# uoo723/PMGT

Hardware: AMD Instinct MI355X
Metric: PMGT pre-train nodes/sec (higher is better)
Workload: dtype bf16; 1 GPU; c2: 7252 nodes / 88606 edges, L=4 H=8 d=256 I=256 S=32 (context=S tokens incl. target), B=1024 targets/GPU/step, 12 sequences/target, dropout 0.1, beta 0.5, clip 5.0, AdamW lr 1e-4 wd 1e-2; parallelism=dp1, global_batch=1024, seq_len=32

## Files before the change

include/pmgt_ops.h:

```cpp
#ifndef PMGT_OPS_H
#define PMGT_OPS_H

#include "pmgt_capi.h"

#ifdef __cplusplus
extern "C" {
#endif

#define PMGT_OPT_TILE_GEMM (1u << 0)
#define PMGT_OPT_VALU_ATTENTION (1u << 1)
#define PMGT_OPT_WAVE_ATTENTION_BWD (1u << 2)
#define PMGT_OPT_NO_SHORTCUT (1u << 3)
#define PMGT_OPT_NO_FUSED_QKVC_ATTENTION (1u << 4)
#define PMGT_OPT_NO_HEAD_MAJOR (1u << 5)
#define PMGT_OPT_NO_TABLE_PROJECTION (1u << 6)
#define PMGT_OPT_NO_SEGMENT_SUM (1u << 7)
#define PMGT_OPT_CONSUMER_QUANT (1u << 8)
#define PMGT_OPT_NO_FUSED_ATTENTION_BWD (1u << 9)
#define PMGT_OPT_STORE_LN_INPUT (1u << 10)
#define PMGT_OPT_EAGER_REDUCE (1u << 11)
#define PMGT_OPT_SIDE_STREAM_REDUCE (1u << 12)
#define PMGT_OPT_UNFUSED_LN (1u << 13)
#define PMGT_OPT_ONE_BUCKET (1u << 14)
#define PMGT_OPT_SMALL_ARENA (1u << 15)
#define PMGT_OPT_NO_ROLE_SPLIT_LN (1u << 16)
#define PMGT_OPT_UNFUSED_LN_BWD (1u << 18)
#define PMGT_OPT_LOCKSTEP_ATTENTION_BWD (1u << 19)
#define PMGT_OPT_SIDE_STREAM_WGRAD (1u << 20)
#define PMGT_OPT_NO_CLS_ONLY_ATTENTION_BWD (1u << 21)
#define PMGT_OPT_NO_BETA_SKIP (1u << 22)
#define PMGT_OPT_NO_VC2_ATTENTION_BWD (1u << 23)
#define PMGT_OPT_NO_TILE_ATTENTION (1u << 17)

void pmgt_launch_trace_reset(void);
int64_t pmgt_launch_trace_count(const char* family);

int pmgt_op_clock_probe(uint64_t* out, int blocks, void* stream);
int64_t pmgt_op_seg_sort_temp_bytes(int M);
int pmgt_op_seg_sort(const int64_t* ids, int M, int n_rows, uint32_t* scratch_keys, uint32_t* scratch_vals, uint32_t* skeys, uint32_t* perm,
                     int* seg_off, void* temp, int64_t temp_bytes, void* stream);
int pmgt_op_quant_rows_e4m3(int src_dtype, const void* src, int64_t lds, int rows, int cols, void* dst, int64_t ldd,
                            float* scale, void* stream);
int pmgt_op_gemm_nt_f8(const void* A, int64_t lda, const int64_t* a_rows, const float* a_row_scale, float a_scale,
                       const void* B, int64_t ldb, const float* b_row_scale, void* C, int64_t ldc, int M, int N, int K,
                       const float* bias, const int* m_dev, void* stream);
int pmgt_op_gemm_tn_f8(const void* P, int64_t ldp, const void* Q8, int64_t ldq, float q_scale, const int64_t* q_rows, int M,
                       int N1, int N2, float* slab, float* out, int accumulate, const int* m_dev, void* stream);
int pmgt_op_qkvc_attention_fwd_f8(const void* x, const void* x8, const float* xscale, const void* w8, const float* wscale, const float* bias, const float* mask,
                                  void* qkvc, void* ctx, int n_seq, int S, int H, int dh, float beta, float drop_p,
                                  uint32_t site1, uint32_t site2, const uint64_t* rng, void* stream);
int pmgt_op_gemm_nt(int dtype, const void* A, int64_t lda, const int64_t* a_rows, const void* B, int64_t ldb, void* C,
                    int64_t ldc, int M, int N, int K, const float* bias, int epilogue, void* aux, int64_t ldaux,
                    const void* residual, int64_t ldr, float drop_p, uint32_t drop_site, const uint64_t* rng,
                    const int* m_dev, uint32_t path_opts, void* stream);
int64_t pmgt_op_gemm_tn_slab_elems(int dtype, int M, int N1, int N2, uint32_t path_opts);
int pmgt_op_gemm_tn(int dtype, const void* P, int64_t ldp, const void* Q, int64_t ldq, const int64_t* q_rows, int M,
                    int N1, int N2, float* slab, float* out, int accumulate, const int* m_dev, uint32_t path_opts, void* stream);
int pmgt_op_gemm_tn_bias(int dtype, const void* P, int64_t ldp, const void* Q, int64_t ldq, int M, int N1, int N2, float* slab,
                         float* out, float* bias_slab, float* bias_out, int perm_d, int perm_dh, uint32_t path_opts, void* stream);
int pmgt_op_colsum(int dtype, const void* Y, int64_t ldy, int M, int N, float* slab, float* out, void* stream);
int pmgt_op_layernorm_fwd(int dtype, const void* x, void* y, float* stats, const float* gamma, const float* beta,
                          int M, int d, float eps, float drop_p, uint32_t drop_site, const uint64_t* rng, void* stream);
int pmgt_op_layernorm_bwd(int dtype, const void* dy, const void* x, const float* stats, const float* gamma, void* dx,
                          void* dx_drop, float* part, float* dgamma_dbeta, int M, int d, float in_drop_p,
                          uint32_t in_site, float out_drop_p, uint32_t out_site, const uint64_t* rng, void* stream);
int pmgt_op_linear(int dtype, const void* A, int64_t lda, const void* B, int64_t ldb, void* C, int64_t ldc, int M, int N, int K,
                   const float* bias, int epilogue, void* aux, int64_t ldaux, const void* residual, int64_t ldr, float drop_p,
                   uint32_t drop_site, const uint64_t* rng, void* ln_out, float* ln_stats, const float* ln_gamma,
                   const float* ln_beta, float ln_eps, uint32_t path_opts, void* stream);
int pmgt_op_linear_ln_bwd(const void* A, int64_t lda, const void* B, int64_t ldb, int M, int N, int K, const void* residual, int64_t ldr,
                          const void* y, const float* stats, const float* gamma, const float* beta, void* dy_tmp, void* dx, void* dx_drop,
                          float drop_p, uint32_t drop_site, const uint64_t* rng, float* part, float* dgamma_dbeta_dbias,
                          uint32_t path_opts, void* stream);
int pmgt_op_linear_rows(int dtype, const void* A, int64_t lda, const int64_t* a_rows, const void* B, int64_t ldb, void* C, int64_t ldc, int M,
                        int N, int K, const float* bias, int epilogue, void* aux, int64_t ldaux, const void* residual, int64_t ldr,
                        int res_gather, float drop_p, uint32_t drop_site, const uint64_t* rng, void* ln_out, float* ln_stats,
                        const float* ln_gamma, const float* ln_beta, float ln_eps, const int* m_dev, uint32_t path_opts, void* stream);
int pmgt_op_layernorm_bwd_rows(int dtype, const void* dy, const void* x, const float* stats, const float* gamma, void* dx,
                               void* dx_drop, float* part, float* dgamma_dbeta, int M, int d, float in_drop_p, uint32_t in_site,
                               float out_drop_p, uint32_t out_site, const uint64_t* rng, const int* m_dev, void* stream);
int pmgt_op_gemm_tn_bias_rows(int dtype, const void* P, int64_t ldp, const void* Q, int64_t ldq, const int64_t* q_rows, int M, int m_for_splits,
                              int N1, int N2, float* slab, float* out, float* bias_slab, float* bias_out, int accumulate, const int* m_dev,
                              uint32_t path_opts, void* stream);
int pmgt_op_qkvc_attention_fwd(const void* x, const void* w, const float* bias, const float* mask, void* qkvc, void* ctx,
                               int n_seq, int S, int H, int dh, float beta, float drop_p, uint32_t site1, uint32_t site2,
                               const uint64_t* rng, void* stream);
int pmgt_op_qkvc_attention_fwd_ex(const void* x, const void* w, const float* bias, const float* mask, void* qkvc, void* ctx,
                                  int n_seq, int S, int H, int dh, float beta, float drop_p, uint32_t site1, uint32_t site2,
                                  const uint64_t* rng, int flags, void* stream);
int pmgt_op_attention_fwd(int dtype, const void* qkvc, const float* mask, void* ctx, float* probs, int n_seq, int S,
                          int H, int dh, float beta, float drop_p, uint32_t site1, uint32_t site2,
                          const uint64_t* rng, uint32_t path_opts, void* stream);
int pmgt_op_attention_bwd(int dtype, const void* qkvc, const float* mask, const void* dctx, void* dqkvc, int n_seq,
                          int S, int H, int dh, float beta, float drop_p, uint32_t site1, uint32_t site2,
                          const uint64_t* rng, uint32_t path_opts, void* stream);
int pmgt_op_attention_bwd_wgrad_parts(int H);
int pmgt_op_attention_bwd_wgrad_vc2_parts(int H);
int pmgt_op_attention_bwd_wgrad(const void* qkvc, const float* mask, const void* dctx, const void* x, void* dqkvc, float* slab,
                                float* bias_slab, int n_seq, int H, float beta, float drop_p, uint32_t site1, uint32_t site2,
                                const uint64_t* rng, int head_major, void* stream);


typedef struct pmgt_embed_args {
    int dtype, phase, M, S, d, nf;
    const void* E;
    const int64_t* e_rows;
    const float *Wa, *ba, *pos, *role, *gamma, *beta;
    float eps;
    float* a;
    void* pre;
    float* stats;
    void* h0;
    float drop_p;
    uint32_t drop_site;
    const uint64_t* rng;
    const void* dh0;
    void* dE;
    void* dF;
    int dF_f32;
    float* part;
} pmgt_embed_args;
int pmgt_op_embed_mix_fwd(const pmgt_embed_args* args, void* stream);
int pmgt_op_embed_mix_bwd(const pmgt_embed_args* args, void* stream);
int pmgt_op_embed_part_elems(int d, int nf);
int pmgt_op_embed_bwd_parts(int M);
int pmgt_op_pos_role_finish(const float* possum, int S, int d, int max_pos, float* dpos, float* drole, int accumulate, void* stream);
int64_t pmgt_op_seg_part_elems(int M, int cols);
int pmgt_op_seg_sum(int in_dtype, int out_dtype, const void* src, int64_t ld, const uint32_t* skeys, const uint32_t* perm, const int* seg_off,
                    int M, int n_rows, int cols, void* out, float* part, void* stream);
int pmgt_op_pair_offsets(const int64_t* num_pairs, int B, int* off, void* stream);
int pmgt_op_nfr_compact(const int64_t* tgt_full, int B, int S, int seq_off, int64_t* rows, int64_t* tids, int* count, void* stream);
int pmgt_op_nfr_generate(const int64_t* ids, int B, int S, int n_nodes, float random_ratio, float mask_ratio, const uint64_t* rng,
                         int64_t* masked_ids, int64_t* tgt_full, void* stream);
int pmgt_op_build_need_rows(int B, int P, int S, const int64_t* nfr_rows, const int* nfr_count, int64_t* rows, int* count, int* inv,
                            int64_t n_tokens, void* stream);
int pmgt_op_dropout_keep(const uint64_t* rng, float p, uint32_t site, int rows, int cols, uint8_t* out, void* stream);
int pmgt_op_gsr(int dtype, const void* h, void* dh, int B, int S, int d, int64_t cls_stride, const int* off, const float* labels,
                float* logits, float* loss_part, void* stream);
int pmgt_op_nfr_diff_parts(int cap);
int pmgt_op_nfr_diff(int dtype, void* pred, const int64_t* tids, const int* count, int cap, int nf, const int* F, const void* const* tables,
                     int tables_f8, const float* scales, float* sse_part, void* stream);
int pmgt_op_loss_finish(const float* gsr_part, int B, const float* sse_part, int nparts, const int* count, int nf, const int* F, int with_nfr,
                        float* out, int* count_out, void* stream);
int pmgt_op_scatter_rows(int dtype, const void* src, const int64_t* rows, const int* count, int cap, int d, void* dst, int add, void* stream);
int pmgt_op_adamw(float* p, const float* g, float* m, float* v, const uint8_t* decay, int64_t n, float lr, float wd, float b1, float b2,
                  float eps, float max_norm, int64_t* step, float* scal, float* part, void* stream);
int pmgt_op_adamw_scheduled(float* p, const float* g, float* m, float* v, const uint8_t* decay, int64_t n, float lr, float wd, float b1,
                            float b2, float eps, float max_norm, int64_t* step, float* scal, float* part, const pmgt_lr_schedule* sched,
                            void* stream);
int pmgt_op_adamw_guarded(float* p, const float* g, float* m, float* v, const uint8_t* decay, int64_t n, float lr, float wd, float b1,
                          float b2, float eps, float max_norm, int64_t* step, float* scal, float* part, const pmgt_lr_schedule* sched,
                          const pmgt_step_guard* guard, void* stream);
int pmgt_op_sgd(float* p, const float* g, const uint8_t* decay, int64_t n, float lr, float wd, float max_norm, int64_t* step, float* scal,
                float* part, const pmgt_lr_schedule* sched, const pmgt_step_guard* guard, void* stream);
#define PMGT_ADAM_MAX_SEGMENTS 8
typedef struct pmgt_adam_segment {
    float* p;
    const float* g;
    float* m;
    float* v;
    const uint8_t* decay;
    int64_t n;
    float lr_scale;
} pmgt_adam_segment;
int pmgt_op_adamw_segments(const pmgt_adam_segment* segments, int count, float lr, float wd, float b1, float b2, float eps, float max_norm,
                           int64_t* step, float* scal, float* part, void* stream);
#define PMGT_OPTIM_ADAMW 0
#define PMGT_OPTIM_SGD   1
int pmgt_op_step_segments(const pmgt_adam_segment* segments, int count, int optim, float lr, float wd, float b1, float b2, float eps,
                          float max_norm, int64_t* step, float* scal, float* part, const pmgt_lr_schedule* sched,
                          const pmgt_step_guard* guard, void* stream);
int pmgt_op_cls_gather(int dtype, const void* last_hidden, int64_t n, int S, int d, float* x, void* stream);
int pmgt_op_cls_scatter(int dtype, const float* d_item, int64_t n, int S, int d, void* d_last, void* stream);
int pmgt_op_eval_append_scores(void* workspace, int64_t capacity, const float* scores, const float* labels, const float* loss, int64_t offset,
                               int64_t n, int64_t n_targets, void* stream);
int pmgt_op_eval_small_max(void);
int pmgt_op_lr_schedule(const pmgt_lr_schedule* sched, float lr, int64_t first_step, int n, float* out, void* stream);
typedef struct pmgt_mirror_desc {
    int64_t src;
    int rows, cols;
    int64_t dst, dst_t, dst_t_hm;
    int hm_d, hm_dh;
    int tile_start;
} pmgt_mirror_desc;
int pmgt_op_mirror(int dtype, const float* params, void* mirror, const pmgt_mirror_desc* desc, int ndesc, int total_tiles, void* stream);

#ifdef __cplusplus
}
#endif
#endif
```

pmgt_amd/_lib.py:

```python
import ctypes as C
import os

from . import _build

c_i64p = C.POINTER(C.c_int64)
c_f32p = C.POINTER(C.c_float)


MAX_FEATS = 4


class PMGTConfigC(C.Structure):
    _fields_ = [("hidden_size", C.c_int), ("num_hidden_layers", C.c_int), ("num_attention_heads", C.c_int),
                ("intermediate_size", C.c_int), ("n_feats", C.c_int), ("feat_sizes", C.c_int * MAX_FEATS),
                ("max_position_embeddings", C.c_int), ("layer_norm_eps", C.c_float), ("beta", C.c_float),
                ("hidden_dropout_prob", C.c_float), ("attention_probs_dropout_prob", C.c_float), ("dtype", C.c_int)]


class TensorsC(C.Structure):
    _fields_ = [("params", C.c_void_p), ("grads", C.c_void_p), ("tables", C.c_void_p * MAX_FEATS),
                ("n_nodes", C.c_int64), ("rng_state", C.c_void_p), ("table_scales", C.c_float * MAX_FEATS)]


class BatchC(C.Structure):
# ... 69 lines not shown
class NcfDropoutC(C.Structure):
    _fields_ = [("rng", C.c_void_p), ("p_emb", C.c_float), ("p_layer", C.c_float * 4)]


class AdamSegmentC(C.Structure):
    _fields_ = [("p", C.c_void_p), ("g", C.c_void_p), ("m", C.c_void_p), ("v", C.c_void_p), ("decay", C.c_void_p), ("n", C.c_int64),
                ("lr_scale", C.c_float)]


ADAM_MAX_SEGMENTS = 8
OPTIMS = ("adamw", "sgd")


class DcnHeadC(C.Structure):
    _fields_ = [("factor_num", C.c_int), ("deep_layers", C.c_int), ("cross_layers", C.c_int), ("use_layer_norm", C.c_int),
                ("layer_norm_eps", C.c_float), ("reserved", C.c_int), ("user_num", C.c_int64), ("item_num", C.c_int64),
                ("params", C.c_void_p), ("grads", C.c_void_p)]


class DcnDropoutC(C.Structure):
    _fields_ = [("rng", C.c_void_p), ("p_emb", C.c_float), ("p_deep", C.c_float * 4), ("p_cross", C.c_float * 6)]


NCF_KINDS = ("MLP", "NeuMF-end")
NCF_MAX_LAYERS, NCF_MAX_USERS = 4, 1 << 20
NCF_FACTORS, NCF_MAX_D = (8, 16, 32, 64), 256
NCF_TRAIN_MAX_PAIRS, NCF_TRAIN_TENSORS = 65536, 13
NCF_MODEL_KINDS, NCF_MODEL_TENSORS = ("MLP", "NeuMF-end", "GMF", "NeuMF-pre"), 22
NCF_SITE_EMB, NCF_SITE_GMF, NCF_SITE_LAYER = 64, 65, 72
DCN_MAX_DEEP, DCN_MAX_CROSS, DCN_TENSORS, DCN_MAX_PAIRS = 4, 6, 38, 65536
DCN_SITE_EMB, DCN_SITE_DEEP, DCN_SITE_CROSS = 64, 72, 80
DCN_SCORE_ROW_STRIDE = 12
DCN_FACTORS, DCN_MAX_E = (8, 16, 32, 64), 256
TOPK_MAX_K, TOPK_FLAG_NAN, TOPK_FLAG_SHORT = 1024, 1, 2
RANK_HELDOUT_CHUNK, RANK_HELDOUT_FLAG_EXCLUDED, RANK_HELDOUT_HEADER_BYTES = 1024, 4, 128
ITEM_GRAPH_MIN_SLOTS, ITEM_GRAPH_MAX_SLOTS = 16, 1024
ITEM_SIM_MAX_D = 1024
HISTORY_AGGS = ("mean", "max")

AVG_MODES = ("swa", "ema")
AVG_STATE_BYTES = 32

STEP_LOG_FLOATS = 8
STEP_LOG_APPLIED, STEP_LOG_SKIPPED, STEP_LOG_APPLIED_NONFINITE = 0, 1, 2

LR_SCHEDULE_TYPES = ("constant", "constant_with_warmup", "linear", "cosine", "cosine_with_restarts", "polynomial")

DTYPE_F32, DTYPE_BF16, DTYPE_FP8 = 0, 1, 2
GRAD_READY_FN = C.CFUNCTYPE(None, C.c_void_p, C.c_int64, C.c_int64)
FLAG_TRAINING, FLAG_BACKWARD, FLAG_ACCUMULATE = 1, 2, 4
EPI_NONE, EPI_GELU, EPI_GELU_GRAD = 0, 1, 2

HIP_SYMBOLS = [
    "pmgt_last_error", "pmgt_abi_version", "pmgt_engine_create", "pmgt_engine_destroy", "pmgt_param_count",
    "pmgt_param_num_entries", "pmgt_param_entry", "pmgt_workspace_bytes", "pmgt_pretrain_step", "pmgt_encode_ids",
    "pmgt_encode_feats", "pmgt_encode_train", "pmgt_encode_backward", "pmgt_optimizer_step", "pmgt_optimizer_step_scheduled", "pmgt_optimizer_step_guarded", "pmgt_profile_begin",
    "pmgt_profile_end", "pmgt_profile_sequence", "pmgt_profile_records", "pmgt_cast_from_f32", "pmgt_cast_to_f32", "pmgt_quantize_e4m3", "pmgt_dequantize_e4m3",
    "pmgt_engine_set_grad_ready_callback", "pmgt_engine_set_option", "pmgt_engine_get_option",
    "pmgt_eval_workspace_bytes", "pmgt_eval_reset", "pmgt_eval_append", "pmgt_eval_reduce",
    "pmgt_weight_average_update", "pmgt_weight_swap",
    "pmgt_rank_workspace_bytes", "pmgt_rank_reset", "pmgt_rank_append", "pmgt_rank_reduce",
    "pmgt_ncf_score", "pmgt_topk_workspace_bytes", "pmgt_topk_rows", "pmgt_rank_heldout", "pmgt_rank_heldout_reduce",
    "pmgt_item_graph_default_slots", "pmgt_item_graph_count", "pmgt_item_graph_fill", "pmgt_item_sim_norms", "pmgt_item_sim_score", "pmgt_history_score",
    "pmgt_knn_score", "pmgt_knn_score_tile",
    "pmgt_ncf_train_layout", "pmgt_ncf_train_workspace_bytes", "pmgt_ncf_train_grad",
    "pmgt_ncf_train_table_workspace_bytes", "pmgt_ncf_train_grad_table", "pmgt_ncf_train_grad_dropout",
    "pmgt_ncf_train_rows_workspace_bytes", "pmgt_ncf_train_grad_rows",
    "pmgt_ncf_model_layout", "pmgt_ncf_model_workspace_bytes", "pmgt_ncf_model_train_grad", "pmgt_ncf_model_score",
    "pmgt_dcn_layout", "pmgt_dcn_workspace_bytes", "pmgt_dcn_forward", "pmgt_dcn_train_grad",
    "pmgt_dcn_train_grad_dropout", "pmgt_dcn_score_rows", "pmgt_dcn_score",
]
OPS_SYMBOLS = [
    "pmgt_op_gemm_nt", "pmgt_op_gemm_tn_slab_elems", "pmgt_op_gemm_tn", "pmgt_op_gemm_tn_bias", "pmgt_op_colsum",
    "pmgt_op_layernorm_fwd", "pmgt_op_layernorm_bwd", "pmgt_op_linear", "pmgt_op_linear_ln_bwd", "pmgt_op_attention_fwd", "pmgt_op_attention_bwd",
    "pmgt_op_qkvc_attention_fwd", "pmgt_op_attention_bwd_wgrad", "pmgt_op_attention_bwd_wgrad_parts",
    "pmgt_op_quant_rows_e4m3", "pmgt_op_gemm_nt_f8", "pmgt_op_gemm_tn_f8", "pmgt_op_qkvc_attention_fwd_f8",
    "pmgt_launch_trace_reset", "pmgt_launch_trace_count", "pmgt_op_seg_sort", "pmgt_op_seg_sort_temp_bytes", "pmgt_op_clock_probe", "pmgt_op_qkvc_attention_fwd_ex", "pmgt_op_attention_bwd_wgrad_vc2_parts",
    "pmgt_op_embed_mix_fwd", "pmgt_op_embed_mix_bwd", "pmgt_op_embed_part_elems", "pmgt_op_embed_bwd_parts", "pmgt_op_pos_role_finish",
    "pmgt_op_seg_part_elems", "pmgt_op_seg_sum", "pmgt_op_pair_offsets", "pmgt_op_nfr_compact", "pmgt_op_gsr", "pmgt_op_nfr_diff_parts",
    "pmgt_op_nfr_diff", "pmgt_op_loss_finish", "pmgt_op_scatter_rows", "pmgt_op_adamw", "pmgt_op_mirror",
    "pmgt_op_adamw_scheduled", "pmgt_op_lr_schedule", "pmgt_op_nfr_generate", "pmgt_op_build_need_rows", "pmgt_op_dropout_keep",
    "pmgt_op_adamw_guarded", "pmgt_op_eval_append_scores", "pmgt_op_eval_small_max",
    "pmgt_op_linear_rows", "pmgt_op_layernorm_bwd_rows", "pmgt_op_gemm_tn_bias_rows",
    "pmgt_op_adamw_segments", "pmgt_op_cls_gather", "pmgt_op_cls_scatter", "pmgt_op_sgd", "pmgt_op_step_segments",
]
OPT = {k: 1 << i for i, k in enumerate((
    "tile_gemm", "valu_attention", "wave_attention_bwd", "no_shortcut", "no_fused_qkvc_attention", "no_head_major",
    "no_table_projection", "no_segment_sum", "consumer_quant", "no_fused_attention_bwd", "store_ln_input", "eager_reduce",
    "side_stream_reduce", "unfused_ln", "one_bucket", "small_arena", "no_role_split_ln", "no_tile_attention", "unfused_ln_bwd", "lockstep_attention_bwd", "side_stream_wgrad", "no_cls_only_attention_bwd", "no_beta_skip", "no_vc2_attention_bwd"))}
SAMPLER_SYMBOLS = [
    "pmgt_sampler_create", "pmgt_sampler_destroy", "pmgt_sampler_last_error", "pmgt_sampler_seed",
    "pmgt_sampler_context", "pmgt_sampler_batch", "pmgt_sampler_batch_mt", "pmgt_sampler_max_pairs",
    "pmgt_sampler_random_sample", "pmgt_sampler_randint", "pmgt_train_valid_split",
]

_hip = None
_sampler = None


def _load(path, what):
    if not os.path.exists(path):
        raise ImportError(f"{what} not built: {path} is missing. Run `python __graft_entry__.py` "
                          f"(or pmgt_amd._build.build_all()); pmgt_amd has no fallback path.")
    try:
        return C.CDLL(path)
    except OSError as e:
        raise ImportError(f"cannot load {what} ({path}): {e}") from e


def hip():
    global _hip
    if _hip is not None:
        return _hip
    import torch
    L = _load(_build.hip_lib_path(), "HIP engine library")
    vp, i, i64, f, u32 = C.c_void_p, C.c_int, C.c_int64, C.c_float, C.c_uint32
    L.pmgt_last_error.restype = C.c_char_p
    L.pmgt_abi_version.restype = i
    L.pmgt_engine_create.restype = vp
    L.pmgt_engine_create.argtypes = [C.POINTER(PMGTConfigC)]
    L.pmgt_engine_destroy.argtypes = [vp]
    L.pmgt_engine_destroy.restype = None
    L.pmgt_param_count.restype = i64
    L.pmgt_param_count.argtypes = [vp]
    L.pmgt_param_num_entries.argtypes = [vp]
    L.pmgt_param_entry.argtypes = [vp, i, C.c_char_p, i, c_i64p, c_i64p, C.POINTER(i), C.POINTER(i), C.POINTER(i)]
    L.pmgt_workspace_bytes.restype = i64
    L.pmgt_workspace_bytes.argtypes = [vp, i, i, i, i]
    L.pmgt_pretrain_step.argtypes = [vp, C.POINTER(TensorsC), C.POINTER(BatchC), C.POINTER(OutputsC), vp, i64, i, vp]
    L.pmgt_encode_ids.argtypes = [vp, C.POINTER(TensorsC), vp, vp, i, i, vp, vp, vp, vp, i64, vp]
    featp = C.POINTER(C.c_void_p)
    L.pmgt_encode_feats.argtypes = [vp, C.POINTER(TensorsC), featp, vp, i, i, vp, vp, vp, vp, i64, vp]
    L.pmgt_encode_train.argtypes = [vp, C.POINTER(TensorsC), vp, featp, vp, i, i, vp, vp, i64, i, vp]
    L.pmgt_encode_backward.argtypes = [vp, C.POINTER(TensorsC), featp, vp, i, i, vp, i64, i, vp]
    L.pmgt_optimizer_step.argtypes = [vp, C.POINTER(TensorsC), C.POINTER(AdamC), vp]
    L.pmgt_optimizer_step_scheduled.argtypes = [vp, C.POINTER(TensorsC), C.POINTER(AdamC), C.POINTER(LrScheduleC), vp]
    L.pmgt_optimizer_step_guarded.argtypes = [vp, C.POINTER(TensorsC), C.POINTER(AdamC), C.POINTER(LrScheduleC), C.POINTER(StepGuardC), vp]
    L.pmgt_profile_begin.argtypes = [vp]
    L.pmgt_profile_end.argtypes = [vp, C.c_char_p, i]
    L.pmgt_profile_sequence.argtypes = [vp, C.c_char_p, i]
    L.pmgt_profile_records.argtypes = [vp, C.c_char_p, i]
    L.pmgt_cast_from_f32.argtypes = [i, vp, vp, i64, vp]
    L.pmgt_cast_to_f32.argtypes = [i, vp, vp, i64, vp]
    L.pmgt_op_gemm_nt.argtypes = [i, vp, i64, vp, vp, i64, vp, i64, i, i, i, vp, i, vp, i64, vp, i64, f, u32, vp, vp, u32, vp]
    L.pmgt_op_gemm_tn_slab_elems.restype = i64
    L.pmgt_op_gemm_tn_slab_elems.argtypes = [i, i, i, i, u32]
    L.pmgt_op_gemm_tn.argtypes = [i, vp, i64, vp, i64, vp, i, i, i, vp, vp, i, vp, u32, vp]
    L.pmgt_op_colsum.argtypes = [i, vp, i64, i, i, vp, vp, vp]
    L.pmgt_op_layernorm_fwd.argtypes = [i, vp, vp, vp, vp, vp, i, i, f, f, u32, vp, vp]
    L.pmgt_op_layernorm_bwd.argtypes = [i, vp, vp, vp, vp, vp, vp, vp, vp, i, i, f, u32, f, u32, vp, vp]
    L.pmgt_op_qkvc_attention_fwd.argtypes = [vp, vp, vp, vp, vp, vp, i, i, i, i, f, f, u32, u32, vp, vp]
    L.pmgt_engine_set_grad_ready_callback.argtypes = [vp, GRAD_READY_FN, vp]
    L.pmgt_engine_set_grad_ready_callback.restype = None
    L.pmgt_engine_set_option.argtypes = [vp, C.c_char_p, i]
    L.pmgt_engine_get_option.argtypes = [vp, C.c_char_p]
    L.pmgt_op_linear.argtypes = [i, vp, i64, vp, i64, vp, i64, i, i, i, vp, i, vp, i64, vp, i64, f, u32, vp, vp, vp, vp, vp, f, u32, vp]
    L.pmgt_launch_trace_count.argtypes = [C.c_char_p]
    L.pmgt_launch_trace_count.restype = C.c_int64
    L.pmgt_launch_trace_reset.restype = None
    L.pmgt_op_clock_probe.argtypes = [vp, i, vp]
    L.pmgt_op_qkvc_attention_fwd_ex.argtypes = [vp, vp, vp, vp, vp, vp, i, i, i, i, f, f, u32, u32, vp, i, vp]
    L.pmgt_op_seg_sort_temp_bytes.argtypes = [i]
    L.pmgt_op_seg_sort_temp_bytes.restype = i64
    L.pmgt_op_seg_sort.argtypes = [vp, i, i, vp, vp, vp, vp, vp, vp, i64, vp]
    L.pmgt_op_linear_ln_bwd.argtypes = [vp, i64, vp, i64, i, i, i, vp, i64, vp, vp, vp, vp, vp, vp, vp, f, u32, vp, vp, vp, u32, vp]
    L.pmgt_op_attention_fwd.argtypes = [i, vp, vp, vp, vp, i, i, i, i, f, f, u32, u32, vp, u32, vp]
    L.pmgt_op_attention_bwd.argtypes = [i, vp, vp, vp, vp, i, i, i, i, f, f, u32, u32, vp, u32, vp]
    L.pmgt_op_attention_bwd_wgrad.argtypes = [vp, vp, vp, vp, vp, vp, vp, i, i, f, f, u32, u32, vp, i, vp]
    L.pmgt_op_attention_bwd_wgrad_parts.argtypes = [i]
    L.pmgt_op_attention_bwd_wgrad_vc2_parts.argtypes = [i]
    L.pmgt_op_gemm_tn_bias.argtypes = [i, vp, i64, vp, i64, i, i, i, vp, vp, vp, vp, i, i, u32, vp]
    L.pmgt_op_linear_rows.argtypes = [i, vp, i64, vp, vp, i64, vp, i64, i, i, i, vp, i, vp, i64, vp, i64, i, f, u32, vp, vp, vp, vp, vp, f, vp, u32, vp]
    L.pmgt_op_layernorm_bwd_rows.argtypes = [i, vp, vp, vp, vp, vp, vp, vp, vp, i, i, f, u32, f, u32, vp, vp, vp]
    L.pmgt_op_gemm_tn_bias_rows.argtypes = [i, vp, i64, vp, i64, vp, i, i, i, i, vp, vp, vp, vp, i, vp, u32, vp]
    L.pmgt_quantize_e4m3.argtypes = [vp, vp, i64, f, vp]
    L.pmgt_dequantize_e4m3.argtypes = [vp, vp, i64, f, vp]
    L.pmgt_op_quant_rows_e4m3.argtypes = [i, vp, i64, i, i, vp, i64, vp, vp]
    L.pmgt_op_gemm_nt_f8.argtypes = [vp, i64, vp, vp, f, vp, i64, vp, vp, i64, i, i, i, vp, vp, vp]
    L.pmgt_op_gemm_tn_f8.argtypes = [vp, i64, vp, i64, f, vp, i, i, i, vp, vp, i, vp, vp]
    L.pmgt_op_qkvc_attention_fwd_f8.argtypes = [vp, vp, vp, vp, vp, vp, vp, vp, vp, i, i, i, i, f, f, u32, u32, vp, vp]
    L.pmgt_op_embed_mix_fwd.argtypes = [C.POINTER(EmbedArgsC), vp]
    L.pmgt_op_embed_mix_bwd.argtypes = [C.POINTER(EmbedArgsC), vp]
    L.pmgt_op_embed_part_elems.argtypes = [i, i]
    L.pmgt_op_embed_bwd_parts.argtypes = [i]
    L.pmgt_op_pos_role_finish.argtypes = [vp, i, i, i, vp, vp, i, vp]
    L.pmgt_op_seg_part_elems.argtypes = [i, i]
    L.pmgt_op_seg_part_elems.restype = i64
    L.pmgt_op_seg_sum.argtypes = [i, i, vp, i64, vp, vp, vp, i, i, i, vp, vp, vp]
    L.pmgt_op_pair_offsets.argtypes = [vp, i, vp, vp]
    L.pmgt_op_nfr_compact.argtypes = [vp, i, i, i, vp, vp, vp, vp]
    L.pmgt_op_gsr.argtypes = [i, vp, vp, i, i, i, i64, vp, vp, vp, vp, vp]
    L.pmgt_op_nfr_diff_parts.argtypes = [i]
    L.pmgt_op_nfr_diff.argtypes = [i, vp, vp, vp, i, i, C.POINTER(i), C.POINTER(vp), i, c_f32p, vp, vp]
    L.pmgt_op_loss_finish.argtypes = [vp, i, vp, i, vp, i, C.POINTER(i), i, vp, vp, vp]
    L.pmgt_op_scatter_rows.argtypes = [i, vp, vp, vp, i, i, vp, i, vp]
    L.pmgt_op_adamw.argtypes = [vp, vp, vp, vp, vp, i64, f, f, f, f, f, f, vp, vp, vp, vp]
    L.pmgt_op_adamw_scheduled.argtypes = [vp, vp, vp, vp, vp, i64, f, f, f, f, f, f, vp, vp, vp, C.POINTER(LrScheduleC), vp]
    L.pmgt_op_adamw_guarded.argtypes = [vp, vp, vp, vp, vp, i64, f, f, f, f, f, f, vp, vp, vp, C.POINTER(LrScheduleC), C.POINTER(StepGuardC), vp]
    L.pmgt_op_lr_schedule.argtypes = [C.POINTER(LrScheduleC), f, i64, i, vp, vp]
    L.pmgt_op_sgd.argtypes = [vp, vp, vp, i64, f, f, f, vp, vp, vp, C.POINTER(LrScheduleC), C.POINTER(StepGuardC), vp]
    L.pmgt_op_mirror.argtypes = [i, vp, vp, C.POINTER(MirrorDescC), i, i, vp]
    L.pmgt_op_nfr_generate.argtypes = [vp, i, i, i, f, f, vp, vp, vp, vp]
    L.pmgt_op_build_need_rows.argtypes = [i, i, i, vp, vp, vp, vp, vp, i64, vp]
    L.pmgt_op_dropout_keep.argtypes = [vp, f, u32, i, i, vp, vp]
    L.pmgt_eval_workspace_bytes.restype = i64
    L.pmgt_eval_workspace_bytes.argtypes = [i64]
    L.pmgt_eval_reset.argtypes = [vp, i64, vp]
    L.pmgt_eval_append.argtypes = [vp, i64, vp, vp, vp, i64, i64, i64, vp]
    L.pmgt_eval_reduce.argtypes = [vp, i64, i64, vp]
    L.pmgt_op_eval_append_scores.argtypes = [vp, i64, vp, vp, vp, i64, i64, i64, vp]
    L.pmgt_op_eval_small_max.argtypes = []
    L.pmgt_weight_average_update.argtypes = [vp, vp, i64, C.POINTER(AvgStepC), vp]
    L.pmgt_weight_swap.argtypes = [vp, vp, i64, vp]
    L.pmgt_rank_workspace_bytes.restype = i64
    L.pmgt_rank_workspace_bytes.argtypes = [i64, i]
    L.pmgt_rank_reset.argtypes = [vp, i64, vp, i, vp, vp, vp]
    L.pmgt_rank_append.argtypes = [vp, i64, vp, vp, vp, i64, i64, i64, vp]
    L.pmgt_rank_reduce.argtypes = [vp, i64, i64, vp]
    L.pmgt_ncf_score.argtypes = [C.POINTER(NcfHeadC), vp, vp, vp, i64, i64, vp, i64, vp]
    L.pmgt_topk_workspace_bytes.restype = i64
    L.pmgt_topk_workspace_bytes.argtypes = [i64, i64]
    L.pmgt_topk_rows.argtypes = [vp, i64, i64, i64, i, vp, vp, vp, i64, i64, vp, vp, vp, vp, vp]
    L.pmgt_rank_heldout.argtypes = [vp, i64, i64, i64, vp, vp, vp, i64, i64, vp, vp, i64, vp, vp, vp]
    L.pmgt_rank_heldout_reduce.argtypes = [vp, vp, vp, vp, i64, i64, i64, vp, i, vp, vp, vp, vp, vp]
    L.pmgt_item_graph_default_slots.argtypes = []
    L.pmgt_item_graph_count.argtypes = [vp, vp, vp, vp, vp, i64, i64, i64, i64, i, vp, vp, vp, i64, vp]
    L.pmgt_item_graph_fill.argtypes = [vp, vp, vp, vp, vp, i64, i64, i64, i64, i, vp, vp, vp, i64, vp, vp, vp, i64, vp]
    L.pmgt_item_sim_norms.argtypes = [vp, i64, i, f, vp, vp]
    L.pmgt_item_sim_score.argtypes = [vp, vp, vp, i64, i64, i, vp, i64, vp]
    L.pmgt_history_score.argtypes = [vp, vp, vp, vp, vp, i64, i64, i64, i, i, vp, i64, vp]
    L.pmgt_knn_score.argtypes = [vp, vp, i64, i, vp, vp, vp, vp, i64, i64, i64, vp, i64, vp]
    L.pmgt_knn_score_tile.argtypes = []
    L.pmgt_ncf_train_layout.restype = i64
    L.pmgt_ncf_train_layout.argtypes = [i, i, i, i64, i64, vp]
    L.pmgt_ncf_train_workspace_bytes.restype = i64
    L.pmgt_ncf_train_workspace_bytes.argtypes = [i, i, i, i64]
    L.pmgt_ncf_train_grad.argtypes = [C.POINTER(NcfTrainC), vp, vp, vp, i64, vp, vp, vp, i64, vp]
    L.pmgt_ncf_train_table_workspace_bytes.restype = i64
    L.pmgt_ncf_train_table_workspace_bytes.argtypes = [i, i, i, i64]
    L.pmgt_ncf_train_grad_table.argtypes = [C.POINTER(NcfTrainC), vp, vp, vp, i64, vp, vp, vp, vp, i64, vp]
    L.pmgt_ncf_train_grad_dropout.argtypes = [C.POINTER(NcfTrainC), vp, vp, vp, i64, vp, vp, vp, C.POINTER(NcfDropoutC), vp, i64, vp]
    L.pmgt_ncf_train_rows_workspace_bytes.restype = i64
    L.pmgt_ncf_train_rows_workspace_bytes.argtypes = [i, i, i, i64]
    L.pmgt_ncf_train_grad_rows.argtypes = [C.POINTER(NcfTrainC), vp, vp, vp, i64, vp, vp, vp, vp, C.POINTER(NcfDropoutC), vp, i64, vp]
    L.pmgt_ncf_model_layout.restype = i64
    L.pmgt_ncf_model_layout.argtypes = [i, i, i, i, i, i64, i64, vp]
    L.pmgt_ncf_model_workspace_bytes.restype = i64
    L.pmgt_ncf_model_workspace_bytes.argtypes = [i, i, i, i, i, i64]
    L.pmgt_ncf_model_train_grad.argtypes = [C.POINTER(NcfModelC), vp, vp, vp, i64, vp, vp, C.POINTER(NcfDropoutC), vp, i64, vp]
    L.pmgt_ncf_model_score.argtypes = [C.POINTER(NcfModelHeadC), vp, vp, vp, i64, i64, vp, i64, vp]
    L.pmgt_op_adamw_segments.argtypes = [C.POINTER(AdamSegmentC), i, f, f, f, f, f, f, vp, vp, vp, vp]
    L.pmgt_op_step_segments.argtypes = [C.POINTER(AdamSegmentC), i, i, f, f, f, f, f, f, vp, vp, vp, C.POINTER(LrScheduleC),
                                        C.POINTER(StepGuardC), vp]
    L.pmgt_op_cls_gather.argtypes = [i, vp, i64, i, i, vp, vp]
    L.pmgt_op_cls_scatter.argtypes = [i, vp, i64, i, i, vp, vp]
    L.pmgt_dcn_layout.restype = i64
    L.pmgt_dcn_layout.argtypes = [i, i, i, i, i64, i64, vp]
    L.pmgt_dcn_workspace_bytes.restype = i64
    L.pmgt_dcn_workspace_bytes.argtypes = [i, i, i, i, i64]
    L.pmgt_dcn_forward.argtypes = [C.POINTER(DcnHeadC), vp, vp, i64, vp, vp, i64, vp]
    L.pmgt_dcn_train_grad.argtypes = [C.POINTER(DcnHeadC), vp, vp, vp, i64, vp, vp, vp, i64, vp]
    L.pmgt_dcn_score_rows.argtypes = [C.POINTER(DcnHeadC), vp, i64, i, vp, vp]
    L.pmgt_dcn_score.argtypes = [C.POINTER(DcnHeadC), vp, vp, vp, vp, vp, vp, i64, i64, vp, i64, vp]
    L.pmgt_dcn_train_grad_dropout.argtypes = [C.POINTER(DcnHeadC), vp, vp, vp, i64, vp, vp, C.POINTER(DcnDropoutC), vp, i64, vp]
    _hip = L
# ... 66 lines not shown
```

pmgt_amd/csrc/common.h:

```cpp
#pragma once
#include <hip/hip_runtime.h>
#include <stdint.h>

#include <atomic>

namespace pmgt {

typedef __bf16 bf16;
typedef __attribute__((ext_vector_type(8))) __bf16 bf16x8;
typedef __attribute__((ext_vector_type(4))) __bf16 bf16x4;
typedef __attribute__((ext_vector_type(4))) float f32x4;
typedef __attribute__((ext_vector_type(4))) uint32_t u32x4;
typedef __attribute__((ext_vector_type(2))) uint32_t u32x2;

constexpr int WAVE = 64;

void set_error(const char* fmt, ...);
#define PMGT_CHECK(cond, code, ...)                                                               \
    do {                                                                                          \
        if (!(cond)) {                                                                            \
            ::pmgt::set_error(__VA_ARGS__);                                                       \
            return (code);                                                                        \
        }                                                                                         \
    } while (0)
#define PMGT_HIP(expr)                                                                            \
    do {                                                                                          \
        hipError_t e__ = (expr);                                                                  \
        if (e__ != hipSuccess) {                                                                  \
            ::pmgt::set_error("%s failed: %s (%s:%d)", #expr, hipGetErrorString(e__), __FILE__,   \
                              __LINE__);                                                          \
            return -100;                                                                          \
        }                                                                                         \
    } while (0)
#define PMGT_SMEM_ATTR(kern, bytes)                                                               \
    do {                                                                                          \
        static std::atomic<uint64_t> done__{0};                                                   \
        int dev__ = 0;                                                                            \
        PMGT_HIP(hipGetDevice(&dev__));                                                           \
        const uint64_t bit__ = 1ull << (dev__ & 63);                                              \
        if (!(done__.load(std::memory_order_acquire) & bit__)) {                                  \
            PMGT_HIP(hipFuncSetAttribute((kern), hipFuncAttributeMaxDynamicSharedMemorySize, (bytes))); \
            done__.fetch_or(bit__, std::memory_order_release);                                    \
        }                                                                                         \
    } while (0)
#define PMGT_LAUNCH_OK()                                                                          \
    do {                                                                                          \
        hipError_t e__ = hipGetLastError();                                                       \
        if (e__ != hipSuccess) {                                                                  \
            ::pmgt::set_error("kernel launch failed: %s (%s:%d)", hipGetErrorString(e__),         \
                              __FILE__, __LINE__);                                                \
            return -101;                                                                          \
        }                                                                                         \
    } while (0)

enum LaunchTag {
    LT_GEMM_WSR = 0, LT_GEMM_WSR_LNB, LT_GEMM_WSR512, LT_GEMM_WS, LT_NT_BIG, LT_NT_BIG_GATHER, LT_NT_BIG_128, LT_NT_LNB, LT_NT_TILE,
    LT_TN_BIG, LT_TN_BIG_GATHER, LT_TN_DMA, LT_TN_DMA_GATHER, LT_TN_TILE, LT_ATTN_TILES_FWD, LT_ATTN_TILES_BWD, LT_QKVC_ATTN_FWD,
    LT_ATTN_BWD_WGRAD, LT_F8_BIG, LT_F8_TILE, LT_F8_WSR512, LT_GEMM_ROWLN, LT_NT_LNF, LT_EMBED_TOK8, LT_QKVC_ATTN_FWD_VC, LT_ATTN_BWD_WGRAD_VC, LT_NT_VC, LT_ATTN_BWD_WGRAD_VC2, LT_COUNT
};
void note_launch(int tag);

template <typename T> __device__ __forceinline__ float to_f(T x);
template <> __device__ __forceinline__ float to_f<float>(float x) { return x; }
template <> __device__ __forceinline__ float to_f<bf16>(bf16 x) { return (float)x; }
template <typename T> __device__ __forceinline__ T from_f(float x);
template <> __device__ __forceinline__ float from_f<float>(float x) { return x; }
template <> __device__ __forceinline__ bf16 from_f<bf16>(float x) { return (bf16)x; }

template <typename T> __device__ __forceinline__ f32x4 load4(const T* p);
template <> __device__ __forceinline__ f32x4 load4<float>(const float* p) { return *(const f32x4*)p; }
template <> __device__ __forceinline__ f32x4 load4<bf16>(const bf16* p) {
    bf16x4 v = *(const bf16x4*)p;
    f32x4 r = {(float)v[0], (float)v[1], (float)v[2], (float)v[3]};
    return r;
}
template <typename T> __device__ __forceinline__ void store4(T* p, f32x4 v);
template <> __device__ __forceinline__ void store4<float>(float* p, f32x4 v) { *(f32x4*)p = v; }
template <> __device__ __forceinline__ void store4<bf16>(bf16* p, f32x4 v) {
    bf16x4 r = {(bf16)v[0], (bf16)v[1], (bf16)v[2], (bf16)v[3]};
    *(bf16x4*)p = r;
}

__device__ __forceinline__ void store_row32(bf16* row_c0, f32x4 v0, f32x4 v1, int q, bool pred) {
    const bf16x4 p0 = {(bf16)v0[0], (bf16)v0[1], (bf16)v0[2], (bf16)v0[3]};
    const bf16x4 p1 = {(bf16)v1[0], (bf16)v1[1], (bf16)v1[2], (bf16)v1[3]};
    typedef uint32_t u32x2_t __attribute__((ext_vector_type(2)));
    u32x2_t a = __builtin_bit_cast(u32x2_t, p0), b = __builtin_bit_cast(u32x2_t, p1);
    uint32_t ax = a[0], ay = a[1], bx = b[0], by = b[1];
    asm volatile("s_nop 1\n\tv_permlane16_swap_b32 %0, %1\n\tv_permlane16_swap_b32 %2, %3" : "+v"(ax), "+v"(bx), "+v"(ay), "+v"(by));
    const int cb = ((q & 1) << 4) | ((q & 2) << 2);
    if (pred) *(u32x4*)(row_c0 + cb) = (u32x4){ax, ay, bx, by};
}

struct DropCfg {
    const uint64_t* rng;
    float p;
    uint32_t site;
};
struct DropKey {
    uint32_t k0, k1, thr;
    float scale;
    bool on;
};
__device__ __forceinline__ uint32_t fmix32(uint32_t h) {
    h ^= h >> 16; h *= 0x85ebca6bu; h ^= h >> 13; h *= 0xc2b2ae35u; h ^= h >> 16;
    return h;
}
__device__ __forceinline__ DropKey make_drop_key(const DropCfg& c) {
    DropKey k;
    k.on = c.p > 0.f;
    k.k0 = k.k1 = k.thr = 0; k.scale = 1.f;
    if (k.on) {
        typedef const __attribute__((address_space(4))) uint64_t* rng_cptr;
        const rng_cptr rp = (rng_cptr)(uintptr_t)c.rng;
        const uint64_t seed = rp[0], step = rp[1];
        k.k0 = fmix32((uint32_t)seed ^ (c.site * 0x9E3779B1u));
        k.k1 = fmix32((uint32_t)(seed >> 32) + (uint32_t)step * 0x7FEB352Du + (uint32_t)(step >> 32) + c.site);
        double t = (double)c.p * 4294967296.0;
        k.thr = t >= 4294967295.0 ? 0xFFFFFFFFu : (uint32_t)t;
        k.scale = 1.f / (1.f - c.p);
    }
    return k;
}
__device__ __forceinline__ void drop_mul4(const DropKey& k, uint32_t row, uint32_t cg, float (&m)[4]) {
    uint32_t x = row * 0x9E3779B1u + cg * 0x85EBCA77u + k.k0;
    x ^= x >> 15; x *= 0x2C1B3C6Du; x ^= x >> 12;
    uint32_t y = x * 0x297A2D39u + k.k1;
    y ^= y >> 15;
    const uint32_t t = k.thr >> 16;
    m[0] = (x & 0xFFFFu) >= t ? k.scale : 0.f;
    m[1] = (x >> 16) >= t ? k.scale : 0.f;
    m[2] = (y & 0xFFFFu) >= t ? k.scale : 0.f;
    m[3] = (y >> 16) >= t ? k.scale : 0.f;
}
__device__ __forceinline__ void drop_keep4(const DropKey& k, uint32_t row, uint32_t cg, bool (&keep)[4]) {
    uint32_t x = row * 0x9E3779B1u + cg * 0x85EBCA77u + k.k0;
    x ^= x >> 15; x *= 0x2C1B3C6Du; x ^= x >> 12;
    uint32_t y = x * 0x297A2D39u + k.k1;
    y ^= y >> 15;
    const uint32_t t = k.thr >> 16;
    keep[0] = (x & 0xFFFFu) >= t;
// ... 51 lines not shown
    if constexpr (sizeof(T) == 2) return gelu_fast_grad(x); else return gelu_erf_grad(x);
}

template <int CTRL> __device__ __forceinline__ float dpp_add(float v) {
    return v + __builtin_bit_cast(float, __builtin_amdgcn_update_dpp(0, __builtin_bit_cast(int, v), CTRL, 0xf, 0xf, false));
}
__device__ __forceinline__ float sum_lanes32(float v) {
    v = dpp_add<0x121>(v);
    v = dpp_add<0x122>(v);
    v = dpp_add<0x124>(v);
    v = dpp_add<0x128>(v);
    float a = v, b = v;
    asm volatile("s_nop 1\n\tv_permlane16_swap_b32 %0, %1" : "+v"(a), "+v"(b));
    return a + b;
}

__device__ __forceinline__ float raw_max(float a, float b) {
    float d;
    asm("v_max_f32 %0, %1, %2" : "=v"(d) : "v"(a), "v"(b));
    return d;
}
__device__ __forceinline__ float max_lanes32(float v) {
    v = raw_max(v, __builtin_bit_cast(float, __builtin_amdgcn_update_dpp(0, __builtin_bit_cast(int, v), 0x121, 0xf, 0xf, false)));
    v = raw_max(v, __builtin_bit_cast(float, __builtin_amdgcn_update_dpp(0, __builtin_bit_cast(int, v), 0x122, 0xf, 0xf, false)));
    v = raw_max(v, __builtin_bit_cast(float, __builtin_amdgcn_update_dpp(0, __builtin_bit_cast(int, v), 0x124, 0xf, 0xf, false)));
    v = raw_max(v, __builtin_bit_cast(float, __builtin_amdgcn_update_dpp(0, __builtin_bit_cast(int, v), 0x128, 0xf, 0xf, false)));
    float x = v, y = v;
    asm volatile("s_nop 1\n\tv_permlane16_swap_b32 %0, %1" : "+v"(x), "+v"(y));
    return raw_max(x, y);
}

__device__ __forceinline__ float wave_sum(float v) {
    v = dpp_add<0xB1>(v);
    v = dpp_add<0x4E>(v);
    v = dpp_add<0x141>(v);
    v = dpp_add<0x140>(v);
    float a = v, b = v;
    asm volatile("s_nop 1\n\tv_permlane16_swap_b32 %0, %1" : "+v"(a), "+v"(b));
    v = a + b;
    a = v; b = v;
    asm volatile("s_nop 1\n\tv_permlane32_swap_b32 %0, %1" : "+v"(a), "+v"(b));
    return a + b;
}
template <int CTRL> __device__ __forceinline__ float dpp_max(float v) {
    return fmaxf(v, __builtin_bit_cast(float, __builtin_amdgcn_update_dpp(0, __builtin_bit_cast(int, v), CTRL, 0xf, 0xf, false)));
}
__device__ __forceinline__ float wave_max(float v) {
    v = dpp_max<0xB1>(v);
    v = dpp_max<0x4E>(v);
    v = dpp_max<0x141>(v);
    v = dpp_max<0x140>(v);
    float a = v, b = v;
    asm volatile("s_nop 1\n\tv_permlane16_swap_b32 %0, %1" : "+v"(a), "+v"(b));
    v = fmaxf(a, b);
    a = v; b = v;
    asm volatile("s_nop 1\n\tv_permlane32_swap_b32 %0, %1" : "+v"(a), "+v"(b));
    return fmaxf(a, b);
}

enum PathOpt : uint32_t {
    OPT_TILE_GEMM = 1u << 0,
    OPT_VALU_ATTENTION = 1u << 1,
    OPT_WAVE_ATTENTION_BWD = 1u << 2,
    OPT_NO_SHORTCUT = 1u << 3,
    OPT_NO_FUSED_QKVC_ATTENTION = 1u << 4,
    OPT_NO_HEAD_MAJOR = 1u << 5,
    OPT_NO_TABLE_PROJECTION = 1u << 6,
    OPT_NO_SEGMENT_SUM = 1u << 7,
    OPT_CONSUMER_QUANT = 1u << 8,
    OPT_NO_FUSED_ATTENTION_BWD = 1u << 9,
    OPT_STORE_LN_INPUT = 1u << 10,
    OPT_EAGER_REDUCE = 1u << 11,
    OPT_SIDE_STREAM_REDUCE = 1u << 12,
    OPT_UNFUSED_LN = 1u << 13,
    OPT_ONE_BUCKET = 1u << 14,
    OPT_SMALL_ARENA = 1u << 15,
    OPT_NO_ROLE_SPLIT_LN = 1u << 16,
    OPT_NO_TILE_ATTENTION = 1u << 17,
    OPT_UNFUSED_LN_BWD = 1u << 18,
    OPT_LOCKSTEP_ATTENTION_BWD = 1u << 19,
    OPT_NO_CLS_ONLY_ATTENTION_BWD = 1u << 21,
    OPT_NO_BETA_SKIP = 1u << 22,
    OPT_NO_VC2_ATTENTION_BWD = 1u << 23,
    OPT_SIDE_STREAM_WGRAD = 1u << 20,
};

inline int cdiv(int a, int b) { return (a + b - 1) / b; }
inline int64_t cdiv64(int64_t a, int64_t b) { return (a + b - 1) / b; }

}
```

pmgt_amd/csrc/engine.hip:

```cpp
#include <stdarg.h>
#include <stdio.h>
#include <string.h>

#include <string>
#include <map>
#include <vector>

#include "../../include/pmgt_ops.h"
#include "attention.h"
#include "fp8.h"
#include "gemm.h"
#include "loss.h"
#include "optim.h"
#include "rowops.h"
#include "segsum.h"

namespace pmgt {

static thread_local char g_err[1024] = "";
void set_error(const char* fmt, ...) {
    va_list ap;
    va_start(ap, fmt);
    vsnprintf(g_err, sizeof(g_err), fmt, ap);
    va_end(ap);
}

static thread_local int64_t g_launch_count[LT_COUNT] = {};
void note_launch(int tag) { if (tag >= 0 && tag < LT_COUNT) ++g_launch_count[tag]; }
static const char* const g_launch_names[LT_COUNT] = {
    "gemm_wsr", "gemm_wsr_lnb", "gemm_wsr512", "gemm_ws", "nt_big", "nt_big_gather", "nt_big_128", "nt_lnb", "nt_tile",
    "tn_big", "tn_big_gather", "tn_dma", "tn_dma_gather", "tn_tile", "attn_tiles_fwd", "attn_tiles_bwd", "qkvc_attn_fwd",
    "attn_bwd_wgrad", "f8_big", "f8_tile", "f8_wsr512", "gemm_rowln", "nt_lnf", "embed_tok8", "qkvc_attn_fwd_vc", "attn_bwd_wgrad_vc", "nt_vc", "attn_bwd_wgrad_vc2"};

static inline int64_t align_up(int64_t x, int64_t a) { return (x + a - 1) / a * a; }

struct Profiler {
    bool on = false;
    struct Rec { const char* name; hipEvent_t a, b; };
    std::vector<Rec> recs;
    std::vector<hipEvent_t> pool;
    hipEvent_t get() {
        if (!pool.empty()) { hipEvent_t e = pool.back(); pool.pop_back(); return e; }
        hipEvent_t e;
        (void)hipEventCreate(&e);
        return e;
    }
    void clear() {
        for (auto& r : recs) { pool.push_back(r.a); pool.push_back(r.b); }
        recs.clear();
    }
};

struct ParamEntry {
    std::string name;
    int64_t offset, numel;
    int rows, cols, decay;
};

struct LayerOff {
    int64_t Wqkvc, bqkvc, Wo, bo, ln1g, ln1b, W1, b1, W2, b2, ln2g, ln2b;
    int64_t mWqkvc, mWqkvcT, mWo, mWoT, mW1, mW1T, mW2, mW2T;
    int64_t mWqkvcT_hm = -1;
    int64_t m8Wqkvc = -1, s8Wqkvc = -1;
};

}

using namespace pmgt;

struct pmgt_engine {
    pmgt_config cfg;
    int d, L, H, I, dh;
    int NF = 0, F[PMGT_MAX_FEATS] = {0, 0, 0, 0}, Fsum = 0, Foff[PMGT_MAX_FEATS] = {0, 0, 0, 0};
    int64_t pos, role, Wf[PMGT_MAX_FEATS], bf, ln_g, ln_b, Wa, ba, Wn, bn, total;
    std::vector<LayerOff> layers;
    std::vector<ParamEntry> entries;
    int64_t mWf[PMGT_MAX_FEATS], mWn, mWnT, mirror_elems;
    bool fp8 = false;
    int64_t m8Wf[PMGT_MAX_FEATS] = {-1, -1, -1, -1}, s8Wf[PMGT_MAX_FEATS] = {-1, -1, -1, -1}, mirror8_bytes = 0, mscale_elems = 0;
    std::vector<QuantDesc> desc8;
    QuantDesc* desc8_dev = nullptr;
    int desc8_rows = 0;
    std::vector<MirrorDesc> desc;
    MirrorDesc* desc_dev = nullptr;
    int mirror_tiles = 0;
    const void* zeros = nullptr;
    pmgt::Profiler prof;
    hipStream_t side = nullptr;
    std::vector<hipEvent_t> sync_ev;
    size_t sync_next = 0;
    uint32_t opts = 0;
    static constexpr uint32_t SCHED_OPTS = OPT_EAGER_REDUCE | OPT_SIDE_STREAM_REDUCE | OPT_ONE_BUCKET | OPT_SMALL_ARENA;
    std::map<const void*, uint32_t> fwd_opts;
    bool overlap() const { return (opts & OPT_SIDE_STREAM_REDUCE) != 0; }
    pmgt_grad_ready_fn grad_cb = nullptr;
    void* grad_cb_user = nullptr;
    bool grad_cb_fine() const { return grad_cb != nullptr && !(overlap() && side != nullptr) && !(opts & OPT_ONE_BUCKET); }
    void grad_ready(int64_t off, int64_t numel) const { if (grad_cb && numel > 0) grad_cb(grad_cb_user, off, numel); }
    void reserve_sync(size_t n) {
        while (sync_ev.size() < n) {
            hipEvent_t ev = nullptr;
            (void)hipEventCreateWithFlags(&ev, hipEventDisableTiming);
            sync_ev.push_back(ev);
        }
    }
    hipEvent_t next_sync() {
        reserve_sync(256);
        return sync_ev[sync_next++ % sync_ev.size()];
    }
};

namespace pmgt {

static int64_t take(int64_t& cur, int64_t n) {
    int64_t o = cur;
// ... 165 lines not shown
    int64_t* need_rows = nullptr;
    int* need_cnt = nullptr;
    int* need_inv = nullptr;
    LayerBufs<T> ctail;
    T *c_dh = nullptr, *c_bB = nullptr, *c_bC = nullptr, *c_bD = nullptr, *c_big = nullptr;
};

static int64_t sort_temp_bytes(int M) {
    static std::map<int, int64_t> cache;
    auto itr = cache.find(M);
    if (itr != cache.end()) return itr->second;
    const int64_t v = seg_sort_temp_bytes(M);
    cache[M] = v;
    return v;
}

static int64_t tn_slab_elems(int dtype, int M, int N1, int N2, uint32_t opts) {
    const int bkm = dtype != PMGT_DTYPE_F32 ? 64 : 32;
    return (int64_t)gemm_tn_pick_splits(M, N1, N2, bkm, opts) * N1 * N2;
}

template <typename T>
static void carve(const pmgt_engine* e, Carver& c, Bufs<T>& b, int Tseq, int S, int B, bool training) {
    const int d = e->d, I = e->I, L = e->L, F = e->Fsum, NF = e->NF;
    const int64_t M = (int64_t)Tseq * S;
    b.rng_snap = c.get<int64_t>(2);
    b.ids = c.get<int64_t>(M);
    b.mask = c.get<float>(M);
    b.mirror = c.get<T>(e->mirror_elems);
    if (e->fp8) {
        b.mirror8 = c.get<char>(e->mirror8_bytes);
        b.mscale = c.get<float>(e->mscale_elems);
        b.x8 = c.get<char>(M * d);
        b.xscale = c.get<float>(M);
    }
    b.E = c.get<T>(M * std::max(NF, 2) * d);
    b.a = c.get<float>(M * NF);
    b.emb_pre = c.get<T>(M * d);
    b.emb_stats = c.get<float>(M * 2);
    b.h0 = c.get<T>(M * d);
    const int nl = training ? L : std::min(L, 2);
    b.layer.resize(L);
    for (int l = 0; l < nl; ++l) {
        LayerBufs<T>& lb = b.layer[l];
        lb.qkvc = c.get<T>(M * 4 * d);
        lb.ctx = c.get<T>(M * d);
        lb.ao_pre = c.get<T>(M * d);
        lb.stats1 = c.get<float>(M * 2);
        lb.u = c.get<T>(M * d);
        lb.ff_pre = c.get<T>(M * I);
        lb.g = c.get<T>(M * I);
        lb.fo_pre = c.get<T>(M * d);
        lb.stats2 = c.get<float>(M * 2);
        lb.hout = c.get<T>(M * d);
    }
    for (int l = nl; l < L; ++l) b.layer[l] = b.layer[l & 1];
    b.off = c.get<int>(B + 1);
    b.gsr_part = c.get<float>(std::max(B, 1));
    b.nfr_count = c.get<int>(4);
    if (!training) return;
    const int cap = B * std::max(S - 1, 1);
    b.bA = c.get<T>(M * d);
    b.bB = c.get<T>(M * d);
    b.bC = c.get<T>(M * d);
    b.bD = c.get<T>(M * d);
    b.big = c.get<T>(M * std::max(I, 4 * d));
    int64_t slab = 0;
    const int dt = e->cfg.dtype;
    slab = std::max(slab, tn_slab_elems(dt, (int)M, 4 * d, d, e->opts));
    slab = std::max(slab, (int64_t)attn_bwd_wgrad_parts(e->H) * 4 * d * d);
    slab = std::max(slab, tn_slab_elems(dt, (int)M, d, d, e->opts));
    slab = std::max(slab, tn_slab_elems(dt, (int)M, I, d, e->opts));
    slab = std::max(slab, tn_slab_elems(dt, (int)M, d, I, e->opts));
    for (int m = 0; m < NF; ++m) slab = std::max(slab, tn_slab_elems(dt, (int)M, d, e->F[m], e->opts));
    slab = std::max(slab, tn_slab_elems(dt, std::max(256, cap / 5), F, d, e->opts));
    b.slab_elems = align_up(slab, 64);
    b.slab = c.get<float>(2 * b.slab_elems);
    int64_t part = 0;
    part = std::max(part, (int64_t)ln_bwd_parts((int)M) * 3 * d);
    part = std::max(part, (int64_t)embed_bwd_parts((int)M) * embed_part_elems(d, NF));
    part = std::max(part, colsum_slab_elems((int)M, std::max(I, 4 * d)));
    part = std::max(part, colsum_slab_elems(Tseq, S * d));
    part = std::max(part, colsum_slab_elems(cap, F));
    part = std::max(part, (int64_t)512 * std::max(std::max(I, 4 * d), F));
    b.part = c.get<float>(part);
    b.part_side_elems = (int64_t)512 * std::max(std::max(I, 4 * d), F);
    b.part_side = c.get<float>(2 * b.part_side_elems);
    b.ln_part_elems = align_up((int64_t)ln_bwd_parts((int)M) * 3 * d, 64);
    b.ln_part = c.get<float>(2 * b.ln_part_elems);
    b.arena_elems = 2 * b.slab_elems + 4 * b.part_side_elems + 2 * b.ln_part_elems + align_up(part, 64);
    if (e->opts & OPT_SMALL_ARENA)
        b.arena_elems = std::max(b.slab_elems + b.part_side_elems, std::max(b.ln_part_elems, align_up(part, 64))) + 128;
    b.arena = c.get<float>(b.arena_elems);
    b.defer = !(e->opts & OPT_EAGER_REDUCE) && !(e->overlap() && e->side != nullptr);
    b.sg_keys = c.get<uint32_t>(M); b.sg_vals = c.get<uint32_t>(M); b.sg_skeys = c.get<uint32_t>(M); b.sg_perm = c.get<uint32_t>(M);
    b.sg_off = c.get<int>(M / 2 + 4);
    b.sg_tmp_bytes = sort_temp_bytes((int)M);
    b.sg_tmp = c.raw(b.sg_tmp_bytes);
    b.sg_part = c.get<float>(seg_part_elems((int)M, 2 * d));
    b.possum = c.get<float>((int64_t)S * d);
    b.sse_part = c.get<float>((int64_t)nfr_diff_parts(cap) * MAX_FEATS);
    b.nfr_masked = c.get<int64_t>((int64_t)B * S);
    b.nfr_tgt = c.get<int64_t>((int64_t)B * S);
    b.nfr_rows = c.get<int64_t>(cap);
    b.nfr_tids = c.get<int64_t>(cap);
    b.pred = c.get<T>((int64_t)cap * F);
    b.dq = c.get<T>((int64_t)cap * d);
    const int64_t R = (int64_t)B + (Tseq - 2 * B) + cap;
    b.rcap = (int)R;
    b.need_rows = c.get<int64_t>(R);
    b.need_cnt = c.get<int>(4);
    b.need_inv = c.get<int>(M);
    b.ctail.qkvc = nullptr; b.ctail.ctx = nullptr;
    b.ctail.ao_pre = c.get<T>(R * d);
    b.ctail.stats1 = c.get<float>(R * 2);
    b.ctail.u = c.get<T>(R * d);
    b.ctail.ff_pre = c.get<T>(R * I);
    b.ctail.g = c.get<T>(R * I);
    b.ctail.fo_pre = c.get<T>(R * d);
    b.ctail.stats2 = c.get<float>(R * 2);
    b.ctail.hout = c.get<T>(R * d);
    b.c_dh = c.get<T>(R * d);
    b.c_bB = c.get<T>(R * d);
    b.c_bC = c.get<T>(R * d);
    b.c_bD = c.get<T>(R * d);
    b.c_big = c.get<T>(R * std::max(I, d));
}

template <typename T> static inline const T* wsel(const pmgt_engine* e, const pmgt_tensors* t, const Bufs<T>& b, int64_t master_off, int64_t mirror_off) {
    if (mirror_off >= 0) return b.mirror + mirror_off;
    return (const T*)(t->params + master_off);
}

static inline DropCfg dropcfg(const pmgt_tensors* t, bool on, float p, int layer, int kind) {
    DropCfg c;
    c.rng = t->rng_state;
    c.p = on ? p : 0.f;
    c.site = site_id(layer, kind);
    return c;
}

#define RUN(x)                                                                                    \
    do {                                                                                          \
        int rc__ = (x);                                                                           \
        if (rc__ != 0) return rc__;                                                               \
    } while (0)
#define RUNP(name, x)                                                                             \
    do {                                                                                          \
        Profiler& pf__ = const_cast<pmgt_engine*>(e)->prof;                                       \
        hipEvent_t ea__ = nullptr, eb__ = nullptr;                                                \
        if (pf__.on) { ea__ = pf__.get(); eb__ = pf__.get(); (void)hipEventRecord(ea__, st); }     \
        int rc__ = (x);                                                                           \
        if (pf__.on) { (void)hipEventRecord(eb__, st); pf__.recs.push_back({name, ea__, eb__}); }  \
        if (rc__ != 0) return rc__;                                                               \
    } while (0)

static void* g_zero_page = nullptr;
static const void* zero_page() {
    if (!g_zero_page) {
        if (hipMalloc(&g_zero_page, 4096) != hipSuccess || hipMemset(g_zero_page, 0, 4096) != hipSuccess) g_zero_page = nullptr;
    }
    return g_zero_page;
}
template <typename T>
static inline bool ln_from_y_applies(const pmgt_engine* e, int Mt, int K, bool compacted) {
    if (sizeof(T) != 2 || compacted || (e->opts & (OPT_STORE_LN_INPUT | OPT_TILE_GEMM | OPT_UNFUSED_LN))) return false;
    if (e->d != 256) return false;
    if (K > 512) return !e->fp8 && gemm_nt_lnf_shape(Mt, 256, K);
    return Mt >= 64 && K >= 64 && (K & (K - 1)) == 0;
}

template <typename T>
static int linear(const pmgt_engine* e, const char* name, const GemmWS& g, hipStream_t st) {
    if constexpr (sizeof(T) == 2) {
        if (g.ln_out && gemm_rowln_ok(g)) {
            RUNP(name, gemm_rowln(g, st));
            return 0;
        }
        if (g.ln_out && gemm_nt_lnf_ok(g)) {
            RUNP(name, gemm_nt_lnf(g, st));
            return 0;
        }
        if (!(g.opts & OPT_TILE_GEMM) && gemm_ws_supported(g)) {
            PMGT_CHECK(!g.skip_c || gemm_ws_fuses_ln(g), -2, "linear: skip_c needs the fused-LayerNorm form");
            RUNP(name, gemm_ws(g, st));
            if (g.ln_out && !gemm_ws_fuses_ln(g))
                RUNP("fwd.layernorm", ln_fwd<T>((const T*)g.C, (T*)g.ln_out, g.ln_stats, g.ln_gamma, g.ln_beta, g.M, g.N, g.ln_eps,
                                                DropCfg{nullptr, 0.f, 0}, st, g.m_dev, g.q8, g.q8_scale));
            return 0;
        }
    }
    PMGT_CHECK(!g.skip_c, -2, "linear: skip_c needs the fused-LayerNorm form");
    RUNP(name, gemm_nt<T>(g, st));
    if (g.ln_out)
        RUNP("fwd.layernorm", ln_fwd<T>((const T*)g.C, (T*)g.ln_out, g.ln_stats, g.ln_gamma, g.ln_beta, g.M, g.N, g.ln_eps,
                                        DropCfg{nullptr, 0.f, 0}, st, g.m_dev, g.q8, g.q8_scale));
    return 0;
}

template <typename T>
static int build_mirrors(const pmgt_engine* e, const pmgt_tensors* t, Bufs<T>& b, hipStream_t st) {
    RUNP("mirror", build_mirror<T>(t->params, b.mirror, e->desc_dev, (int)e->desc.size(), e->mirror_tiles, st));
    if (e->fp8) RUNP("mirror", quant_params_e4m3(t->params, e->desc8_dev, (int)e->desc8.size(), e->desc8_rows, b.mirror8, b.mscale, st));
    return 0;
}

template <typename T>
static inline bool embed_recomputes(const pmgt_engine* e, bool table_mode) {
    return table_mode && !(e->opts & OPT_NO_SEGMENT_SUM) && e->d == 256 && sizeof(T) == 2;
}

template <typename T>
static inline bool fused_qa_applies(const pmgt_engine* e, int Tseq, int S, bool want_probs) {
    if (sizeof(T) != 2 || (e->opts & (OPT_NO_FUSED_QKVC_ATTENTION | OPT_TILE_GEMM | OPT_VALU_ATTENTION)) || want_probs) return false;
    return S == 32 && e->dh == 32 && (e->d == 256 || e->d == 128) && e->H % 2 == 0 && Tseq >= 2;
}

template <typename T>
static inline bool vc_only_applies(const pmgt_engine* e, int Tseq, int S, bool want_probs) {
    if (e->cfg.beta != 1.f || e->fp8 || e->H % 4 != 0 || (e->opts & (OPT_NO_BETA_SKIP | OPT_NO_FUSED_ATTENTION_BWD))) return false;
    return fused_qa_applies<T>(e, Tseq, S, want_probs) && attn_bwd_wgrad_shape_ok(Tseq, S, e->dh, e->H);
}

static inline bool use_table_projection(const pmgt_engine* e, const pmgt_tensors* t, int64_t n_tokens, bool by_ids) {
    return by_ids && !(e->opts & OPT_NO_TABLE_PROJECTION) && t->n_nodes > 0 && (t->n_nodes + 2) * std::max(2, e->NF) <= n_tokens;
}

template <typename T>
static int encoder_forward(const pmgt_engine* e, const pmgt_tensors* t, Bufs<T>& b, int Tseq, int S, const int64_t* ids,
                           const void* const* feats, const float* mask, bool train, T* hidden_states,
                           float* attn_probs, hipStream_t st, bool shortcut = false, int n_cls_only = 0) {
    const int d = e->d, I = e->I, L = e->L, H = e->H, NF = e->NF;
    const int M = Tseq * S;
    const float* P = t->params;
    PMGT_CHECK(S <= e->cfg.max_position_embeddings, -2, "sequence length %d exceeds max_position_embeddings %d", S,
               e->cfg.max_position_embeddings);
    const float pd = e->cfg.hidden_dropout_prob, pa = e->cfg.attention_probs_dropout_prob;
    const int64_t n_rows = t->n_nodes + 2;
    const bool table_mode = use_table_projection(e, t, M, ids != nullptr);
    b.e_by_id = table_mode;
    PMGT_CHECK(!e->fp8 || ids != nullptr, -3, "fp8 mode gathers e4m3 feature rows by node id: pre-gathered feature tensors are not supported");
    for (int mod = 0; mod < NF && e->fp8; ++mod) {
        GemmF8 g; g.opts = e->opts;
        const int F = e->F[mod];
        g.A = t->tables[mod]; g.lda = F; g.a_rows = table_mode ? nullptr : ids;
        g.a_scale = t->table_scales[mod];
        g.B = b.mirror8 + e->m8Wf[mod]; g.ldb = F; g.b_row_scale = b.mscale + e->s8Wf[mod];
        g.C = b.E + mod * d; g.ldc = NF * d;
        g.M = table_mode ? (int)n_rows : M; g.N = d; g.K = F;
        g.bias = P + e->bf + mod * d;
        RUNP("fwd.gemm_featproj", gemm_nt_f8(g, st));
    }
    for (int mod = 0; mod < NF && !e->fp8; ++mod) {
        GemmNT g; g.opts = e->opts;
        const int F = e->F[mod];
        if (ids) { g.A = t->tables[mod]; g.a_rows = table_mode ? nullptr : ids; }
        else g.A = feats[mod];
        g.lda = F;
        g.B = wsel<T>(e, t, b, e->Wf[mod], e->mWf[mod]);
        g.ldb = F;
        g.C = b.E + mod * d; g.ldc = NF * d;
        g.M = table_mode ? (int)n_rows : M; g.N = d; g.K = F;
        g.bias = P + e->bf + mod * d;
        RUNP("fwd.gemm_featproj", gemm_nt<T>(g, st));
    }
    {
        EmbedMix m;
        m.S = S; m.d = d; m.nf = NF; m.Wa = P + e->Wa; m.ba = P + e->ba; m.pos = P + e->pos; m.role = P + e->role;
        m.gamma = P + e->ln_g; m.beta = P + e->ln_b; m.eps = e->cfg.layer_norm_eps;
        m.a = b.a; m.stats = b.emb_stats; m.h0 = b.h0;
        m.drop = dropcfg(t, train, pd, -1, SITE_EMB);
        const bool pq = e->fp8 && !(e->opts & OPT_CONSUMER_QUANT);
        if (table_mode && !(e->opts & OPT_NO_SEGMENT_SUM)) {
            T* F_all = b.E + n_rows * NF * d;
            m.phase = 1; m.M = (int)n_rows; m.E = b.E; m.pre = F_all;
            RUNP("fwd.embed_mix", embed_mix_fwd<T>(m, st));
            m.phase = 2; m.M = M; m.E = F_all; m.e_rows = ids; m.pre = embed_recomputes<T>(e, true) ? nullptr : b.emb_pre;
            if (pq) { m.q8 = b.x8; m.q8_scale = b.xscale; }
            RUNP("fwd.embed_mix", embed_mix_fwd<T>(m, st));
        } else {
            m.M = M; m.E = b.E; m.e_rows = table_mode ? ids : nullptr; m.pre = b.emb_pre;
            if (pq) { m.q8 = b.x8; m.q8_scale = b.xscale; }
            RUNP("fwd.embed_mix", embed_mix_fwd<T>(m, st));
        }
    }
    bool x8_ok = e->fp8 && !(e->opts & OPT_CONSUMER_QUANT);
    if (hidden_states) PMGT_HIP(hipMemcpyAsync(hidden_states, b.h0, (size_t)M * d * sizeof(T), hipMemcpyDeviceToDevice, st));
    const T* hin = b.h0;
    for (int l = 0; l < L; ++l) {
        const LayerOff& o = e->layers[l];
        LayerBufs<T>& lb = b.layer[l];
        bool fused = false;
// ... 374 lines not shown
                PMGT_CHECK(abw_ok || !b.qkvc_vc, -2, "beta == 1 skip: the forward left Q / K unwritten but the fused attention backward does not apply here");
                if (b.qkvc_vc && b.qkvc_hm && !vc_dgrad_kmap) PMGT_HIP(hipMemsetAsync(b.big, 0, (size_t)M * 4 * d * sizeof(T), st));
                if (abw_ok && b.defer && attn_bwd_wgrad_vc2_supported(w)) {
                    const int parts2 = attn_bwd_wgrad_vc2_parts(H);
                    PMGT_CHECK((int64_t)parts2 * 2 * d * d <= b.arena_elems, -4, "partial-sum arena too small for the two-heads-per-step attention backward");
                    RUN(take_partials2<T>(e, b, (int64_t)parts2 * 2 * d * d, &w.slab, (int64_t)parts2 * 2 * d, &w.bias_slab, st));
                    RUNP("bwd.attention_wgrad", attn_bwd_wgrad_vc2(w, st));
                    RUN(queue_reduce<T>(e, b, w.slab, parts2, (int64_t)2 * d * d, G + o.Wqkvc + (int64_t)2 * d * d, acc, st));
                    RUN(queue_reduce<T>(e, b, w.bias_slab, parts2, 2 * d, G + o.bqkvc + 2 * d, acc, st));
                    if (!acc) {
                        PMGT_HIP(hipMemsetAsync(G + o.Wqkvc, 0, (size_t)2 * d * d * sizeof(float), st));
                        PMGT_HIP(hipMemsetAsync(G + o.bqkvc, 0, (size_t)2 * d * sizeof(float), st));
                    }
                    fused_bw = true;
                } else if (abw_ok && b.defer) {
                    RUN(take_partials2<T>(e, b, (int64_t)parts * 4 * d * d, &w.slab, (int64_t)parts * 4 * d, &w.bias_slab, st));
                    RUNP("bwd.attention_wgrad", attn_bwd_wgrad(w, st));
                    RUN(queue_reduce<T>(e, b, w.slab, parts, (int64_t)4 * d * d, G + o.Wqkvc, acc, st));
                    RUN(queue_reduce<T>(e, b, w.bias_slab, parts, 4 * d, G + o.bqkvc, acc, st));
                    fused_bw = true;
                } else if (abw_ok) {
                    ++b.wg_idx;
                    RUN(sr.acquire(b.wg_done[slot]));
                    RUNP("bwd.attention_wgrad", attn_bwd_wgrad(w, st));
                    hipStream_t rs = st;
                    RUN(sr.begin(&rs));
                    RUNP("bwd.slab_reduce", slab_reduce(w.slab, parts, (int64_t)4 * d * d, G + o.Wqkvc, acc, rs));
                    RUNP("bwd.slab_reduce", slab_reduce(w.bias_slab, parts, 4 * d, G + o.bqkvc, acc, rs));
                    RUN(sr.end(b.wg_done[slot]));
                    fused_bw = true;
                }
            }
            if (!fused_bw) RUNP("bwd.attention", attn_bwd<T>(a, st));
        }
        if (!fused_bw)
            RUN(wgrad<T>("bwd.wgrad_qkvc", e, b, b.big, 4 * d, hin, d, nullptr, M, M, 4 * d, d, G + o.Wqkvc, acc, nullptr, st, G + o.bqkvc,
                         b.qkvc_hm ? d : 0, b.qkvc_hm ? e->dh : 0));
        RUN(flush_reduces<T>(e, b, st));
        if (e->grad_cb_fine()) e->grad_ready(o.Wqkvc, (l + 1 < L ? e->layers[l + 1].Wqkvc : e->Wn) - o.Wqkvc);
        {
            GemmNT g; g.opts = e->opts;
            g.A = b.big; g.lda = 4 * d; g.B = b.mirror + (b.qkvc_hm ? o.mWqkvcT_hm : o.mWqkvcT); g.ldb = 4 * d; g.C = b.bA; g.ldc = d;
            g.M = M; g.N = d; g.K = 4 * d; g.res = sc ? nullptr : b.bB; g.ldr = d;
            if (b.qkvc_vc && vc_dgrad_kmap) { g.kmap_vc = 1; g.K = 2 * d; }
            else if (b.qkvc_vc && !b.qkvc_hm) { g.A = b.big + 2 * d; g.B = b.mirror + o.mWqkvcT + 2 * d; g.K = 2 * d; }
            bool with_ln = false;
            if constexpr (sizeof(T) == 2) {
                if (l >= 1 && b.defer && ln_from_y_applies<T>(e, M, I, false) && (!sc || b.need_inv != nullptr)) {
                    const LayerOff& on = e->layers[l - 1];
                    GemmNT f = g;
                    f.C = b.bB;
                    if (sc) { f.res = gB; f.ldr = d; f.lnb_res_inv = b.need_inv; }
                    f.lnb_y = b.layer[l - 1].hout; f.lnb_ldy = d; f.lnb_stats = b.layer[l - 1].stats2; f.lnb_gamma = P + on.ln2g; f.lnb_beta = P + on.ln2b;
                    f.lnb_dx_drop = dd ? b.bC : nullptr; f.lnb_lddx = d; f.lnb_drop = dropcfg(t, train, pd, l - 1, SITE_FO);
                    if (gemm_nt_lnb_ok(f)) {
                        const int parts = gemm_nt_lnb_parts(M);
                        RUN(take_partials<T>(e, b, (int64_t)parts * 3 * d, &f.lnb_part, st));
                        RUNP("bwd.dgrad_qkvc_lnb", gemm_nt_lnb(f, st));
                        RUN(queue_reduce<T>(e, b, f.lnb_part, parts, 3 * d, G + on.ln2g, acc, st));
                        with_ln = ln2_done = true;
                    }
                }
            }
            if (!with_ln) {
                RUNP("bwd.dgrad_qkvc", gemm_nt<T>(g, st));
                if (sc) RUN(scatter_rows<T>(gB, b.need_rows, b.need_cnt, Mt, d, b.bA, st, true));
            }
        }
    }
    {
        EmbedMix m;
        m.S = S; m.d = d; m.nf = NF; m.Wa = P + e->Wa; m.gamma = P + e->ln_g; m.a = b.a;
        m.stats = b.emb_stats; m.drop = dropcfg(t, train, pd, -1, SITE_EMB);
        m.part = b.part;
        const int pe = embed_part_elems(d, NF);
        const bool by_node = b.e_by_id && !(e->opts & OPT_NO_SEGMENT_SUM);
        PMGT_CHECK(!e->fp8 || feats == nullptr, -3, "fp8 mode: pre-gathered feature tensors are not supported");
        if (by_node) {
            const int n_rows = (int)t->n_nodes + 2;
            m.phase = 2; m.M = M; m.dh0 = b.bA; m.pre = b.emb_pre; m.dF = b.bB;
            if (embed_recomputes<T>(e, true)) {
                m.pre = nullptr; m.E = b.E + (int64_t)n_rows * NF * d; m.e_rows = b.ids; m.pos = P + e->pos; m.role = P + e->role;
            }
            if (b.defer) RUN(take_partials<T>(e, b, (int64_t)embed_bwd_parts(M) * pe, &m.part, st));
            RUNP("bwd.embed_mix", embed_mix_bwd<T>(m, st));
            if (b.defer) RUN(queue_reduce<T>(e, b, m.part, embed_bwd_parts(M), pe, G + e->ln_g, acc, st));
            else RUNP("bwd.slab_reduce", slab_reduce(b.part, embed_bwd_parts(M), pe, G + e->ln_g, acc, st));
            RUNP("bwd.colsum", colsum<T>(b.bB, (int64_t)S * d, Tseq, S * d, b.part, b.possum, false, nullptr, st));
            RUN(pos_role_finish(b.possum, S, d, e->cfg.max_position_embeddings, G + e->pos, G + e->role, acc, st));
            if (b.sort_done) PMGT_HIP(hipStreamWaitEvent(st, b.sort_done, 0));
            else RUNP("bwd.segsum_featproj", seg_sort(b.ids, M, n_rows, b.sg_keys, b.sg_vals, b.sg_skeys, b.sg_perm, b.sg_off, b.sg_tmp, b.sg_tmp_bytes, st));
            RUNP("bwd.segsum_featproj", (seg_sum<T, float>(b.bB, d, b.sg_skeys, b.sg_perm, b.sg_off, M, n_rows, d, (float*)b.bC, b.sg_part, st)));
            m.phase = 1; m.M = n_rows; m.E = b.E; m.e_rows = nullptr; m.dF = b.bC; m.dF_f32 = true; m.dE = b.bD;
            m.part = b.part;
            if (b.defer) RUN(take_partials<T>(e, b, (int64_t)embed_bwd_parts(n_rows) * pe, &m.part, st));
            RUNP("bwd.embed_mix", embed_mix_bwd<T>(m, st));
            if (b.defer) RUN(queue_reduce<T>(e, b, m.part, embed_bwd_parts(n_rows), pe, G + e->ln_g, true, st));
            else RUNP("bwd.slab_reduce", slab_reduce(b.part, embed_bwd_parts(n_rows), pe, G + e->ln_g, true, st));
            for (int mod = 0; mod < NF; ++mod)
                RUN(wgrad<T>("bwd.wgrad_featproj", e, b, b.bD + mod * d, NF * d, (const T*)t->tables[mod], e->F[mod], nullptr, n_rows, n_rows, d, e->F[mod],
                             G + e->Wf[mod], acc, nullptr, st, G + e->bf + mod * d, 0, 0, e->fp8 ? t->table_scales[mod] : 0.f));
        } else {
            m.M = M; m.E = b.E; m.e_rows = b.e_by_id ? b.ids : nullptr; m.pre = b.emb_pre;
            m.dh0 = b.bA; m.dE = b.big; m.dF = b.bB;
            if (b.defer) RUN(take_partials<T>(e, b, (int64_t)embed_bwd_parts(M) * pe, &m.part, st));
            RUNP("bwd.embed_mix", embed_mix_bwd<T>(m, st));
            if (b.defer) RUN(queue_reduce<T>(e, b, m.part, embed_bwd_parts(M), pe, G + e->ln_g, acc, st));
            else RUNP("bwd.slab_reduce", slab_reduce(b.part, embed_bwd_parts(M), pe, G + e->ln_g, acc, st));
            RUNP("bwd.colsum", colsum<T>(b.bB, (int64_t)S * d, Tseq, S * d, b.part, b.possum, false, nullptr, st));
            RUN(pos_role_finish(b.possum, S, d, e->cfg.max_position_embeddings, G + e->pos, G + e->role, acc, st));
            for (int mod = 0; mod < NF; ++mod)
                RUN(wgrad<T>("bwd.wgrad_featproj", e, b, b.big + mod * d, NF * d, feats ? (const T*)feats[mod] : (const T*)t->tables[mod], e->F[mod],
                             feats ? nullptr : b.ids, M, M, d, e->F[mod], G + e->Wf[mod], acc, nullptr, st, G + e->bf + mod * d, 0, 0,
                             e->fp8 ? t->table_scales[mod] : 0.f));
        }
    }
    RUN(flush_reduces<T>(e, b, st));
    RUN(join_side_all<T>(e, b, st));
    if (e->grad_cb_fine()) e->grad_ready(0, L > 0 ? e->layers[0].Wqkvc : e->Wn);
    else if (e->grad_cb) e->grad_ready(0, whole_buffer ? e->total : e->Wn);
    return 0;
}

template <typename T>
static int pretrain_step(pmgt_engine* e, const pmgt_tensors* t, const pmgt_batch* bt, const pmgt_outputs* o, void* ws,
                         int64_t ws_bytes, int flags, hipStream_t st) {
    const bool train = flags & PMGT_FLAG_TRAINING, bwd = flags & PMGT_FLAG_BACKWARD, acc = flags & PMGT_FLAG_ACCUMULATE;
    const int B = bt->n_targets, Pn = bt->n_pairs, S = bt->seq_len, d = e->d, F = e->Fsum;
    PMGT_CHECK(B > 0 && S > 0, -2, "pretrain_step: empty batch");
    PMGT_CHECK(!bwd || train, -2, "pretrain_step: BACKWARD requires TRAINING (the workspace keeps activations only then)");
    PMGT_CHECK(Pn > 0 && bt->pair_ids && bt->labels && bt->num_pairs, -2,
               "labels must be passed, when set pair_node_inputs (pmgt/pmgt/models.py:66-72)");
    const int Tseq = B + Pn + (train ? B : 0);
    Carver c(ws);
    Bufs<T> b;
    carve<T>(e, c, b, Tseq, S, B, train);
    PMGT_CHECK(c.cur <= ws_bytes, -4, "workspace too small: need %lld bytes, got %lld", (long long)c.cur, (long long)ws_bytes);
    const int64_t bs = (int64_t)B * S, ps = (int64_t)Pn * S;
    {
        CopyJob cj[8];
        int nc = 0;
        cj[nc++] = CopyJob{bt->tgt_ids, b.ids, bs * 8};
        cj[nc++] = CopyJob{bt->tgt_mask, b.mask, bs * 4};
        cj[nc++] = CopyJob{bt->pair_ids, b.ids + bs, ps * 8};
        cj[nc++] = CopyJob{bt->pair_mask, b.mask + bs, ps * 4};
        if (train) {
            cj[nc++] = CopyJob{bt->tgt_mask, b.mask + bs + ps, bs * 4};
            if (bt->nfr_masked_ids) {
                PMGT_CHECK(bt->nfr_targets, -2, "nfr_targets must accompany nfr_masked_ids");
                cj[nc++] = CopyJob{bt->nfr_masked_ids, b.ids + bs + ps, bs * 8};
                cj[nc++] = CopyJob{bt->nfr_targets, b.nfr_tgt, bs * 8};
            }
        }
        RUN(multi_copy(cj, nc, st));
    }
    if (train) {
        if (!bt->nfr_masked_ids)
            RUN(nfr_generate(bt->tgt_ids, B, S, (int)t->n_nodes, bt->random_node_ratio, bt->mask_node_ratio, t->rng_state,
                             b.ids + bs + ps, b.nfr_tgt, st));
        RUN(nfr_compact(b.nfr_tgt, B, S, B + Pn, b.nfr_rows, b.nfr_tids, b.nfr_count, st));
    }
    b.sort_done = nullptr;
    if (bwd && use_table_projection(e, t, (int64_t)Tseq * S, true) && !(e->opts & OPT_NO_SEGMENT_SUM) && e->side) {
        hipEvent_t ev = e->next_sync();
        PMGT_HIP(hipEventRecord(ev, st));
        PMGT_HIP(hipStreamWaitEvent(e->side, ev, 0));
        RUN(seg_sort(b.ids, Tseq * S, (int)t->n_nodes + 2, b.sg_keys, b.sg_vals, b.sg_skeys, b.sg_perm, b.sg_off, b.sg_tmp, b.sg_tmp_bytes, e->side));
        b.sort_done = e->next_sync();
        PMGT_HIP(hipEventRecord(b.sort_done, e->side));
    }
    RUN(build_mirrors<T>(e, t, b, st));
    const bool sc = train && !(e->opts & OPT_NO_SHORTCUT) && o->last_hidden == nullptr;
    if (sc) RUN(build_need_rows(B, Pn, S, b.nfr_rows, b.nfr_count, b.need_rows, b.need_cnt, st, b.need_inv, (int64_t)Tseq * S));
    RUN(encoder_forward<T>(e, t, b, Tseq, S, b.ids, nullptr, b.mask, train, (T*)nullptr, (float*)nullptr, st, sc, B + Pn));
    T* hL = sc ? b.ctail.hout : b.layer[e->L - 1].hout;
// ... 344 lines not shown
                    int64_t ldc, int M, int N, int K, const float* bias, int epilogue, void* aux, int64_t ldaux,
                    const void* residual, int64_t ldr, float drop_p, uint32_t drop_site, const uint64_t* rng, const int* m_dev,
                    uint32_t path_opts, void* stream) {
    GemmNT g; g.opts = path_opts;
    g.A = A; g.lda = lda; g.a_rows = a_rows; g.B = B; g.ldb = ldb; g.C = C; g.ldc = ldc; g.M = M; g.N = N; g.K = K;
    g.bias = bias; g.epi = epilogue; g.aux = aux; g.ldaux = ldaux; g.res = residual; g.ldr = ldr;
    g.drop = DropCfg{rng, rng ? drop_p : 0.f, drop_site}; g.m_dev = m_dev;
    if (dtype == PMGT_DTYPE_BF16) return gemm_nt<bf16>(g, (hipStream_t)stream);
    return gemm_nt<float>(g, (hipStream_t)stream);
}

int64_t pmgt_op_gemm_tn_slab_elems(int dtype, int M, int N1, int N2, uint32_t path_opts) { return tn_slab_elems(dtype, M, N1, N2, path_opts); }

int pmgt_op_gemm_tn(int dtype, const void* P, int64_t ldp, const void* Q, int64_t ldq, const int64_t* q_rows, int M, int N1,
                    int N2, float* slab, float* out, int accumulate, const int* m_dev, uint32_t path_opts, void* stream) {
    GemmTN g; g.opts = path_opts;
    g.P = P; g.ldp = ldp; g.Q = Q; g.ldq = ldq; g.q_rows = q_rows; g.M = M; g.N1 = N1; g.N2 = N2; g.slab = slab; g.m_dev = m_dev;
    g.zeros = zero_page();
    g.splits = gemm_tn_pick_splits(M, N1, N2, dtype == PMGT_DTYPE_BF16 ? 64 : 32, path_opts);
    int rc = dtype == PMGT_DTYPE_BF16 ? gemm_tn<bf16>(g, (hipStream_t)stream) : gemm_tn<float>(g, (hipStream_t)stream);
    if (rc) return rc;
    return slab_reduce(slab, g.splits, (int64_t)N1 * N2, out, accumulate != 0, (hipStream_t)stream);
}

int pmgt_op_gemm_tn_bias(int dtype, const void* P, int64_t ldp, const void* Q, int64_t ldq, int M, int N1, int N2, float* slab,
                         float* out, float* bias_slab, float* bias_out, int perm_d, int perm_dh, uint32_t path_opts, void* stream) {
    GemmTN g; g.opts = path_opts;
    g.P = P; g.ldp = ldp; g.Q = Q; g.ldq = ldq; g.M = M; g.N1 = N1; g.N2 = N2; g.slab = slab; g.bias_slab = bias_slab;
    g.zeros = zero_page(); g.perm_d = perm_d; g.perm_dh = perm_dh;
    g.splits = gemm_tn_pick_splits(M, N1, N2, dtype != PMGT_DTYPE_F32 ? 64 : 32, path_opts);
    PMGT_CHECK(g.splits <= 512, -2, "pmgt_op_gemm_tn_bias: bias_slab holds at most 512 splits");
    int rc = dtype != PMGT_DTYPE_F32 ? gemm_tn<bf16>(g, (hipStream_t)stream) : gemm_tn<float>(g, (hipStream_t)stream);
    if (rc) return rc;
    rc = slab_reduce(slab, g.splits, (int64_t)N1 * N2, out, false, (hipStream_t)stream);
    if (rc || !bias_slab) return rc;
    return slab_reduce(bias_slab, g.splits, N1, bias_out, false, (hipStream_t)stream);
}

int pmgt_op_clock_probe(uint64_t* out, int blocks, void* stream) { return clock_probe(out, blocks, (hipStream_t)stream); }
int64_t pmgt_op_seg_sort_temp_bytes(int M) { return seg_sort_temp_bytes(M); }
int pmgt_op_seg_sort(const int64_t* ids, int M, int n_rows, uint32_t* scratch_keys, uint32_t* scratch_vals, uint32_t* skeys, uint32_t* perm,
                     int* seg_off, void* temp, int64_t temp_bytes, void* stream) {
    return seg_sort(ids, M, n_rows, scratch_keys, scratch_vals, skeys, perm, seg_off, temp, temp_bytes, (hipStream_t)stream);
}

int pmgt_op_colsum(int dtype, const void* Y, int64_t ldy, int M, int N, float* slab, float* out, void* stream) {
    if (dtype == PMGT_DTYPE_BF16) return colsum<bf16>((const bf16*)Y, ldy, M, N, slab, out, false, nullptr, (hipStream_t)stream);
    return colsum<float>((const float*)Y, ldy, M, N, slab, out, false, nullptr, (hipStream_t)stream);
}

int pmgt_op_layernorm_fwd(int dtype, const void* x, void* y, float* stats, const float* gamma, const float* beta, int M,
                          int d, float eps, float drop_p, uint32_t drop_site, const uint64_t* rng, void* stream) {
    DropCfg dc{rng, rng ? drop_p : 0.f, drop_site};
    if (dtype == PMGT_DTYPE_BF16) return ln_fwd<bf16>((const bf16*)x, (bf16*)y, stats, gamma, beta, M, d, eps, dc, (hipStream_t)stream);
    return ln_fwd<float>((const float*)x, (float*)y, stats, gamma, beta, M, d, eps, dc, (hipStream_t)stream);
}

int pmgt_op_layernorm_bwd(int dtype, const void* dy, const void* x, const float* stats, const float* gamma, void* dx,
                          void* dx_drop, float* part, float* dgamma_dbeta, int M, int d, float in_drop_p, uint32_t in_site,
                          float out_drop_p, uint32_t out_site, const uint64_t* rng, void* stream) {
    DropCfg di{rng, rng ? in_drop_p : 0.f, in_site}, dout{rng, rng ? out_drop_p : 0.f, out_site};
    int rc;
    if (dtype == PMGT_DTYPE_BF16)
        rc = ln_bwd<bf16>((const bf16*)dy, (const bf16*)x, stats, gamma, (bf16*)dx, (bf16*)dx_drop, part, M, d, di, dout, (hipStream_t)stream);
    else
        rc = ln_bwd<float>((const float*)dy, (const float*)x, stats, gamma, (float*)dx, (float*)dx_drop, part, M, d, di, dout, (hipStream_t)stream);
    if (rc) return rc;
    return slab_reduce(part, ln_bwd_parts(M), 3 * d, dgamma_dbeta, false, (hipStream_t)stream);
}

static AttnArgs mk_attn(const void* qkvc, const float* mask, int n_seq, int S, int H, int dh, float beta, float drop_p,
                        uint32_t s1, uint32_t s2, const uint64_t* rng, uint32_t path_opts = 0) {
    AttnArgs a; a.opts = path_opts;
    a.qkvc = qkvc; a.mask = mask; a.Tseq = n_seq; a.S = S; a.H = H; a.dh = dh; a.beta = beta;
    a.drop1 = DropCfg{rng, rng ? drop_p : 0.f, s1};
    a.drop2 = DropCfg{rng, rng ? drop_p : 0.f, s2};
    return a;
}

static_assert(PMGT_OPT_TILE_GEMM == OPT_TILE_GEMM && PMGT_OPT_VALU_ATTENTION == OPT_VALU_ATTENTION && PMGT_OPT_WAVE_ATTENTION_BWD == OPT_WAVE_ATTENTION_BWD &&
              PMGT_OPT_NO_SHORTCUT == OPT_NO_SHORTCUT && PMGT_OPT_NO_FUSED_QKVC_ATTENTION == OPT_NO_FUSED_QKVC_ATTENTION && PMGT_OPT_NO_HEAD_MAJOR == OPT_NO_HEAD_MAJOR &&
              PMGT_OPT_NO_TABLE_PROJECTION == OPT_NO_TABLE_PROJECTION && PMGT_OPT_NO_SEGMENT_SUM == OPT_NO_SEGMENT_SUM && PMGT_OPT_CONSUMER_QUANT == OPT_CONSUMER_QUANT &&
              PMGT_OPT_NO_FUSED_ATTENTION_BWD == OPT_NO_FUSED_ATTENTION_BWD && PMGT_OPT_STORE_LN_INPUT == OPT_STORE_LN_INPUT && PMGT_OPT_EAGER_REDUCE == OPT_EAGER_REDUCE &&
              PMGT_OPT_SIDE_STREAM_REDUCE == OPT_SIDE_STREAM_REDUCE && PMGT_OPT_UNFUSED_LN == OPT_UNFUSED_LN && PMGT_OPT_ONE_BUCKET == OPT_ONE_BUCKET && PMGT_OPT_SMALL_ARENA == OPT_SMALL_ARENA && PMGT_OPT_NO_ROLE_SPLIT_LN == OPT_NO_ROLE_SPLIT_LN && PMGT_OPT_NO_TILE_ATTENTION == OPT_NO_TILE_ATTENTION,
              "include/pmgt_ops.h and csrc/common.h disagree on the option bits");
static uint32_t option_bit(const char* key) {
    static const struct { const char* name; uint32_t bit; } tab[] = {
        {"tile_gemm", OPT_TILE_GEMM}, {"valu_attention", OPT_VALU_ATTENTION}, {"wave_attention_bwd", OPT_WAVE_ATTENTION_BWD},
        {"no_shortcut", OPT_NO_SHORTCUT}, {"no_fused_qkvc_attention", OPT_NO_FUSED_QKVC_ATTENTION}, {"no_head_major", OPT_NO_HEAD_MAJOR},
        {"no_table_projection", OPT_NO_TABLE_PROJECTION}, {"no_segment_sum", OPT_NO_SEGMENT_SUM}, {"consumer_quant", OPT_CONSUMER_QUANT},
        {"no_fused_attention_bwd", OPT_NO_FUSED_ATTENTION_BWD}, {"store_ln_input", OPT_STORE_LN_INPUT}, {"eager_reduce", OPT_EAGER_REDUCE},
        {"side_stream_reduce", OPT_SIDE_STREAM_REDUCE}, {"unfused_ln", OPT_UNFUSED_LN}, {"one_bucket", OPT_ONE_BUCKET}, {"small_arena", OPT_SMALL_ARENA}, {"no_role_split_ln", OPT_NO_ROLE_SPLIT_LN}, {"no_tile_attention", OPT_NO_TILE_ATTENTION}, {"unfused_ln_bwd", OPT_UNFUSED_LN_BWD}, {"lockstep_attention_bwd", OPT_LOCKSTEP_ATTENTION_BWD}, {"side_stream_wgrad", OPT_SIDE_STREAM_WGRAD}, {"no_cls_only_attention_bwd", OPT_NO_CLS_ONLY_ATTENTION_BWD}, {"no_beta_skip", OPT_NO_BETA_SKIP}, {"no_vc2_attention_bwd", OPT_NO_VC2_ATTENTION_BWD}};
    for (const auto& t : tab)
        if (key && strcmp(key, t.name) == 0) return t.bit;
    return 0;
}
int pmgt_engine_set_option(pmgt_engine* e, const char* key, int value) {
    PMGT_CHECK(e != nullptr, -2, "pmgt_engine_set_option: NULL engine");
    const uint32_t bit = option_bit(key);
    PMGT_CHECK(bit != 0, -2, "pmgt_engine_set_option: unknown option '%s'", key ? key : "(null)");
    e->opts = value ? (e->opts | bit) : (e->opts & ~bit);
    return 0;
}
void pmgt_launch_trace_reset(void) { for (auto& c : g_launch_count) c = 0; }
int64_t pmgt_launch_trace_count(const char* family) {
    for (int i = 0; i < LT_COUNT; ++i)
        if (family && strcmp(family, g_launch_names[i]) == 0) return g_launch_count[i];
    set_error("pmgt_launch_trace_count: unknown kernel family '%s'", family ? family : "(null)");
    return -1;
}
int pmgt_engine_get_option(const pmgt_engine* e, const char* key) {
    PMGT_CHECK(e != nullptr, -2, "pmgt_engine_get_option: NULL engine");
    const uint32_t bit = option_bit(key);
    PMGT_CHECK(bit != 0, -2, "pmgt_engine_get_option: unknown option '%s'", key ? key : "(null)");
    return (e->opts & bit) ? 1 : 0;
}
void pmgt_engine_set_grad_ready_callback(pmgt_engine* e, pmgt_grad_ready_fn cb, void* user) {
    if (e) { e->grad_cb = cb; e->grad_cb_user = user; }
}

int pmgt_op_linear(int dtype, const void* A, int64_t lda, const void* B, int64_t ldb, void* C, int64_t ldc, int M, int N, int K,
                   const float* bias, int epilogue, void* aux, int64_t ldaux, const void* residual, int64_t ldr, float drop_p,
                   uint32_t drop_site, const uint64_t* rng, void* ln_out, float* ln_stats, const float* ln_gamma,
                   const float* ln_beta, float ln_eps, uint32_t path_opts, void* stream) {
    PMGT_CHECK(A && B && C, -2, "pmgt_op_linear: NULL operand (A, B and C are required)");
    PMGT_CHECK(epilogue == 0 || aux, -2, "pmgt_op_linear: epilogue %d needs aux", epilogue);
    GemmWS g; g.opts = path_opts;
    g.A = A; g.lda = lda; g.B = B; g.ldb = ldb; g.C = C; g.ldc = ldc; g.M = M; g.N = N; g.K = K;
    g.bias = bias; g.epi = epilogue; g.aux = aux; g.ldaux = ldaux; g.res = residual; g.ldr = ldr;
    g.drop = DropCfg{rng, rng ? drop_p : 0.f, drop_site};
    g.ln_out = ln_out; g.ln_stats = ln_stats; g.ln_gamma = ln_gamma; g.ln_beta = ln_beta; g.ln_eps = ln_eps;
    pmgt_engine dummy;
    const pmgt_engine* e = &dummy;
    hipStream_t st = (hipStream_t)stream;
    if (dtype == PMGT_DTYPE_BF16) return linear<bf16>(e, "op.linear", g, st);
    return linear<float>(e, "op.linear", g, st);
}

int pmgt_op_linear_ln_bwd(const void* A, int64_t lda, const void* B, int64_t ldb, int M, int N, int K, const void* residual, int64_t ldr,
                          const void* y, const float* stats, const float* gamma, const float* beta, void* dy_tmp, void* dx, void* dx_drop,
                          float drop_p, uint32_t drop_site, const uint64_t* rng, float* part, float* dgamma_dbeta_dbias,
                          uint32_t path_opts, void* stream) {
    hipStream_t st = (hipStream_t)stream;
    GemmWS g; g.opts = path_opts;
    g.A = A; g.lda = lda; g.B = B; g.ldb = ldb; g.C = dx; g.ldc = N; g.M = M; g.N = N; g.K = K; g.res = residual; g.ldr = ldr;
    g.lnb_y = y; g.lnb_ldy = N; g.lnb_stats = stats; g.lnb_gamma = gamma; g.lnb_beta = beta;
    g.lnb_dx_drop = dx_drop; g.lnb_lddx = N; g.lnb_drop = DropCfg{rng, rng ? drop_p : 0.f, drop_site};
    g.lnb_part = part;
    pmgt_engine dummy;
    const pmgt_engine* e = &dummy;
    if (gemm_wsr_lnb_ok(g)) {
        RUN(gemm_wsr_lnb(g, st));
        return slab_reduce(part, gemm_wsr_lnb_parts(M), 3 * N, dgamma_dbeta_dbias, false, st);
    }
    if (gemm_nt_lnb_ok(g)) {
        RUN(gemm_nt_lnb(g, st));
        return slab_reduce(part, gemm_nt_lnb_parts(M), 3 * N, dgamma_dbeta_dbias, false, st);
    }
    g.C = dy_tmp;
    RUN(linear<bf16>(e, "op.linear", g, st));
    RUN(ln_bwd<bf16>((const bf16*)dy_tmp, (const bf16*)y, stats, gamma, (bf16*)dx, (bf16*)dx_drop, part, M, N, DropCfg{nullptr, 0.f, 0}, g.lnb_drop, st, nullptr, beta));
    return slab_reduce(part, ln_bwd_parts(M), 3 * N, dgamma_dbeta_dbias, false, st);
}

int pmgt_op_attention_fwd(int dtype, const void* qkvc, const float* mask, void* ctx, float* probs, int n_seq, int S, int H,
                          int dh, float beta, float drop_p, uint32_t site1, uint32_t site2, const uint64_t* rng, uint32_t path_opts, void* stream) {
    AttnArgs a = mk_attn(qkvc, mask, n_seq, S, H, dh, beta, drop_p, site1, site2, rng, path_opts);
    a.ctx = ctx; a.probs = probs;
    if (dtype == PMGT_DTYPE_BF16) return attn_fwd<bf16>(a, (hipStream_t)stream);
    return attn_fwd<float>(a, (hipStream_t)stream);
}

int pmgt_op_qkvc_attention_fwd(const void* x, const void* w, const float* bias, const float* mask, void* qkvc, void* ctx, int n_seq, int S,
                               int H, int dh, float beta, float drop_p, uint32_t site1, uint32_t site2, const uint64_t* rng, void* stream) {
    QkvcAttn f;
// ... 94 lines not shown
```

pmgt_amd/csrc/rowops.h:

```cpp
#pragma once
#include "common.h"

namespace pmgt {

template <typename T>
int ln_fwd(const T* x, T* y, float* stats, const float* gamma, const float* beta, int M, int d, float eps,
           DropCfg out_drop, hipStream_t st, const int* m_dev = nullptr, void* q8 = nullptr, float* q8_scale = nullptr);
template <typename T>
int ln_bwd(const T* dy, const T* x, const float* stats, const float* gamma, T* dx, T* dx_drop, float* part,
           int M, int d, DropCfg in_drop, DropCfg out_drop, hipStream_t st, const int* m_dev = nullptr, const float* beta_y = nullptr);
__host__ __device__ inline int ln_bwd_rows(int M) { (void)M; return 64; }
inline int ln_bwd_parts(int M) { return cdiv(M, ln_bwd_rows(M)); }

struct EmbedMix {
    int M = 0, S = 0, d = 0;
    int nf = 2;
    const void* E = nullptr;
    const int64_t* e_rows = nullptr;
    int phase = 0;
    bool dF_f32 = false;
    const float* Wa = nullptr;
    const float* ba = nullptr;
    const float* pos = nullptr;
    const float* role = nullptr;
    const float* gamma = nullptr;
    const float* beta = nullptr;
    float eps = 1e-12f;
    float* a = nullptr;
    void* pre = nullptr;
    float* stats = nullptr;
    void* h0 = nullptr;
    void* q8 = nullptr;
    float* q8_scale = nullptr;
    DropCfg drop = {nullptr, 0.f, 0};
    const void* dh0 = nullptr;
    void* dE = nullptr;
    void* dF = nullptr;
    float* part = nullptr;
};
__host__ __device__ inline int embed_part_elems(int d, int nf) { return (2 + nf * nf) * d + 4; }
template <typename T> int embed_mix_fwd(const EmbedMix& e, hipStream_t st);
template <typename T> int embed_mix_bwd(const EmbedMix& e, hipStream_t st);
inline int embed_bwd_parts(int M) { return cdiv(M, ln_bwd_rows(M)); }
int pos_role_finish(const float* possum, int S, int d, int max_pos, float* dpos, float* drole, bool accumulate,
                    hipStream_t st);

}
```

pmgt_amd/csrc/rowops.hip:

```cpp
#include "fp8.h"
#include "rowops.h"

namespace pmgt {

template <int NCH> __device__ __forceinline__ bool ch_ok(int lane, int i, int nch) { return lane + 64 * i < nch; }

__device__ __forceinline__ float sum4(f32x4 v) { return (v[0] + v[1]) + (v[2] + v[3]); }

template <typename T, int NCH>
__global__ __launch_bounds__(256) void ln_fwd_kernel(const T* __restrict__ x, T* __restrict__ y, float* __restrict__ stats,
                                                     const float* __restrict__ gamma, const float* __restrict__ beta,
                                                     int M, int d, float eps, DropCfg drop, const int* m_dev, char* __restrict__ q8,
                                                     float* __restrict__ q8_scale) {
    const int lane = threadIdx.x & 63, wave = threadIdx.x >> 6;
    const int m = blockIdx.x * 4 + wave;
    if (m_dev) M = min(M, *m_dev);
    if (m >= M) return;
    const int nch = d >> 2;
    const T* xr = x + (int64_t)m * d;
    f32x4 v[NCH];
    float s = 0.f;
#pragma unroll
    for (int i = 0; i < NCH; ++i) {
        const int ch = lane + 64 * i;
        v[i] = ch < nch ? load4<T>(xr + 4 * ch) : (f32x4){0.f, 0.f, 0.f, 0.f};
        s += sum4(v[i]);
    }
    const float mean = wave_sum(s) / (float)d;
    float ss = 0.f;
#pragma unroll
    for (int i = 0; i < NCH; ++i) {
        if (lane + 64 * i < nch) {
            f32x4 t = v[i] - mean;
            ss += sum4(t * t);
        }
    }
    const float rstd = 1.f / sqrtf(wave_sum(ss) / (float)d + eps);
    if (lane == 0) { stats[2 * (int64_t)m] = mean; stats[2 * (int64_t)m + 1] = rstd; }
    const DropKey dk = make_drop_key(drop);
    f32x4 oq[NCH];
    float mx = 0.f;
#pragma unroll
    for (int i = 0; i < NCH; ++i) {
        const int ch = lane + 64 * i;
        oq[i] = (f32x4){0.f, 0.f, 0.f, 0.f};
        if (ch < nch) {
            f32x4 g = *(const f32x4*)(gamma + 4 * ch), b = *(const f32x4*)(beta + 4 * ch);
            f32x4 o = (v[i] - mean) * rstd * g + b;
            if (dk.on) {
{ float dm[4]; drop_mul4(dk, (uint32_t)m, (uint32_t)ch, dm);
#pragma unroll
                    for (int e = 0; e < 4; ++e) o[e] *= dm[e]; }
            }
            store4<T>(y + (int64_t)m * d + 4 * ch, o);
#pragma unroll
            for (int e = 0; e < 4; ++e) { oq[i][e] = to_f<T>(from_f<T>(o[e])); mx = fmaxf(mx, fabsf(oq[i][e])); }
        }
    }
    if (q8) {
        mx = wave_max(mx);
        const float inv = mx > 0.f ? E4M3_MAX / mx : 1.f;
        if (lane == 0) q8_scale[m] = mx > 0.f ? mx / E4M3_MAX : 1.f;
#pragma unroll
        for (int i = 0; i < NCH; ++i) {
            const int ch = lane + 64 * i;
            if (ch < nch) {
                int w = 0;
                w = __builtin_amdgcn_cvt_pk_fp8_f32(__builtin_amdgcn_fmed3f(oq[i][0] * inv, -E4M3_MAX, E4M3_MAX),
                                                    __builtin_amdgcn_fmed3f(oq[i][1] * inv, -E4M3_MAX, E4M3_MAX), w, false);
                w = __builtin_amdgcn_cvt_pk_fp8_f32(__builtin_amdgcn_fmed3f(oq[i][2] * inv, -E4M3_MAX, E4M3_MAX),
                                                    __builtin_amdgcn_fmed3f(oq[i][3] * inv, -E4M3_MAX, E4M3_MAX), w, true);
                *(int*)(q8 + (int64_t)m * d + 4 * ch) = w;
            }
        }
    }
}

template <typename T>
int ln_fwd(const T* x, T* y, float* stats, const float* gamma, const float* beta, int M, int d, float eps,
           DropCfg out_drop, hipStream_t st, const int* m_dev, void* q8v, float* q8_scale) {
    char* q8 = (char*)q8v;
    if (M <= 0) return 0;
    PMGT_CHECK(d % 4 == 0 && d <= 1024, -2, "ln_fwd: hidden size %d must be a multiple of 4 and <= 1024", d);
    dim3 grid(cdiv(M, 4)), block(256);
// ... 317 lines not shown
template <typename T>
__global__ __launch_bounds__(256) void embed_tok8_fwd_kernel(EmbedMix p) {
    static_assert(sizeof(T) == 2, "bf16 only");
    constexpr int R = TOK_R, d = 256;
    const int lane = threadIdx.x & 63, hl = lane & 31, hs = lane >> 5;
    const int S = p.S, Tq = p.M / S;
    const int w = blockIdx.x * 4 + (threadIdx.x >> 6);
    if (w >= tok_tasks(p.M, S)) return;
    const TokTask tk = tok_task(w, S, hs);
    int64_t er[R];
#pragma unroll
    for (int k = 0; k < R; ++k) er[k] = p.e_rows[(int64_t)min(tk.q0 + k, Tq - 1) * S + tk.s];
    bf16x8 x[R];
#pragma unroll
    for (int k = 0; k < R; ++k) x[k] = *(const bf16x8*)((const bf16*)p.E + er[k] * d + 8 * hl);
    f32x4 ps[2], rl[2], gam[2], bet[2];
#pragma unroll
    for (int c = 0; c < 2; ++c) {
        ps[c] = *(const f32x4*)(p.pos + (int64_t)tk.s * d + 8 * hl + 4 * c);
        rl[c] = *(const f32x4*)(p.role + (tk.s > 0 ? d : 0) + 8 * hl + 4 * c);
        gam[c] = *(const f32x4*)(p.gamma + 8 * hl + 4 * c);
        bet[c] = *(const f32x4*)(p.beta + 8 * hl + 4 * c);
    }
    const DropKey dk = make_drop_key(p.drop);
#pragma unroll
    for (int k = 0; k < R; ++k) {
        const bool ok = tk.sv && tk.q0 + k < Tq;
        const int64_t m = (int64_t)min(tk.q0 + k, Tq - 1) * S + tk.s;
        float v[8];
        tok_sum(x[k], ps, rl, v);
        if (p.pre && ok) {
            bf16x8 o;
#pragma unroll
            for (int j = 0; j < 8; ++j) o[j] = (bf16)v[j];
            *(bf16x8*)((bf16*)p.pre + m * d + 8 * hl) = o;
        }
        float sm = 0.f;
#pragma unroll
        for (int j = 0; j < 8; ++j) { v[j] = (float)(bf16)v[j]; sm += v[j]; }
        const float mean = half_sum(sm) / (float)d;
        float sq = 0.f;
#pragma unroll
        for (int j = 0; j < 8; ++j) { v[j] -= mean; sq += v[j] * v[j]; }
        const float rstd = 1.f / sqrtf(half_sum(sq) / (float)d + p.eps);
        if (hl == 0 && ok) { p.stats[2 * m] = mean; p.stats[2 * m + 1] = rstd; }
        float o[8];
#pragma unroll
        for (int j = 0; j < 8; ++j) o[j] = v[j] * rstd * gam[j >> 2][j & 3] + bet[j >> 2][j & 3];
        if (dk.on) {
#pragma unroll
            for (int c = 0; c < 2; ++c) {
                float dm[4];
                drop_mul4(dk, (uint32_t)m, (uint32_t)(2 * hl + c), dm);
#pragma unroll
                for (int e = 0; e < 4; ++e) o[4 * c + e] *= dm[e];
            }
        }
        bf16x8 ob;
#pragma unroll
        for (int j = 0; j < 8; ++j) ob[j] = (bf16)o[j];
        if (ok) *(bf16x8*)((bf16*)p.h0 + m * d + 8 * hl) = ob;
        if (p.q8) {
            float oq[8], mx = 0.f;
#pragma unroll
            for (int j = 0; j < 8; ++j) { oq[j] = (float)ob[j]; mx = fmaxf(mx, fabsf(oq[j])); }
            mx = half_max(mx);
            const float inv = mx > 0.f ? E4M3_MAX / mx : 1.f;
            if (hl == 0 && ok) p.q8_scale[m] = mx > 0.f ? mx / E4M3_MAX : 1.f;
            int wq[2];
#pragma unroll
            for (int c = 0; c < 2; ++c) {
                int w_ = 0;
                w_ = __builtin_amdgcn_cvt_pk_fp8_f32(__builtin_amdgcn_fmed3f(oq[4 * c] * inv, -E4M3_MAX, E4M3_MAX),
                                                     __builtin_amdgcn_fmed3f(oq[4 * c + 1] * inv, -E4M3_MAX, E4M3_MAX), w_, false);
                w_ = __builtin_amdgcn_cvt_pk_fp8_f32(__builtin_amdgcn_fmed3f(oq[4 * c + 2] * inv, -E4M3_MAX, E4M3_MAX),
                                                     __builtin_amdgcn_fmed3f(oq[4 * c + 3] * inv, -E4M3_MAX, E4M3_MAX), w_, true);
                wq[c] = w_;
            }
            if (ok) *(int2*)((char*)p.q8 + m * d + 8 * hl) = make_int2(wq[0], wq[1]);
        }
    }
}

template <typename T>
__global__ __launch_bounds__(256) void embed_tok8_bwd_kernel(EmbedMix p) {
    static_assert(sizeof(T) == 2, "bf16 only");
    extern __shared__ float red[];
    constexpr int R = TOK_R, d = 256;
    const int lane = threadIdx.x & 63, hl = lane & 31, hs = lane >> 5, wave = threadIdx.x >> 6;
    const int S = p.S, Tq = p.M / S;
    const int ntask = tok_tasks(p.M, S);
    const DropKey ik = make_drop_key(p.drop);
    f32x4 gam[2];
#pragma unroll
    for (int c = 0; c < 2; ++c) gam[c] = *(const f32x4*)(p.gamma + 8 * hl + 4 * c);
    float dgam[8], dbet[8];
#pragma unroll
    for (int j = 0; j < 8; ++j) dgam[j] = dbet[j] = 0.f;
    for (int w = blockIdx.x * 4 + wave; w < ntask; w += gridDim.x * 4) {
        const TokTask tk = tok_task(w, S, hs);
        int64_t er[R];
#pragma unroll
        for (int k = 0; k < R; ++k) er[k] = p.e_rows[(int64_t)min(tk.q0 + k, Tq - 1) * S + tk.s];
        bf16x8 x[R], dy[R];
        float mean[R], rstd[R];
#pragma unroll
        for (int k = 0; k < R; ++k) {
            const int64_t m = (int64_t)min(tk.q0 + k, Tq - 1) * S + tk.s;
            x[k] = *(const bf16x8*)((const bf16*)p.E + er[k] * d + 8 * hl);
            dy[k] = *(const bf16x8*)((const bf16*)p.dh0 + m * d + 8 * hl);
            mean[k] = p.stats[2 * m];
            rstd[k] = p.stats[2 * m + 1];
        }
        f32x4 ps[2], rl[2];
#pragma unroll
        for (int c = 0; c < 2; ++c) {
            ps[c] = *(const f32x4*)(p.pos + (int64_t)tk.s * d + 8 * hl + 4 * c);
            rl[c] = *(const f32x4*)(p.role + (tk.s > 0 ? d : 0) + 8 * hl + 4 * c);
        }
#pragma unroll
        for (int k = 0; k < R; ++k) {
            const bool ok = tk.sv && tk.q0 + k < Tq;
            const int64_t m = (int64_t)min(tk.q0 + k, Tq - 1) * S + tk.s;
            float v[8], g[8], dyv[8];
            tok_sum(x[k], ps, rl, v);
#pragma unroll
            for (int j = 0; j < 8; ++j) dyv[j] = ok ? (float)dy[k][j] : 0.f;
            if (ik.on) {
#pragma unroll
                for (int c = 0; c < 2; ++c) {
                    float dm[4];
                    drop_mul4(ik, (uint32_t)m, (uint32_t)(2 * hl + c), dm);
#pragma unroll
                    for (int e = 0; e < 4; ++e) dyv[4 * c + e] *= dm[e];
                }
            }
            float sg = 0.f, sgx = 0.f;
#pragma unroll
            for (int j = 0; j < 8; ++j) {
                v[j] = ((float)(bf16)v[j] - mean[k]) * rstd[k];
                g[j] = dyv[j] * gam[j >> 2][j & 3];
                dgam[j] += dyv[j] * v[j];
                dbet[j] += dyv[j];
                sg += g[j];
                sgx += g[j] * v[j];
            }
            sg = half_sum(sg) * (1.f / (float)d);
            sgx = half_sum(sgx) * (1.f / (float)d);
            bf16x8 o;
#pragma unroll
            for (int j = 0; j < 8; ++j) o[j] = (bf16)((g[j] - sg - v[j] * sgx) * rstd[k]);
            if (ok) *(bf16x8*)((bf16*)p.dF + m * d + 8 * hl) = o;
        }
    }
    for (int hw = 0; hw < 8; ++hw) {
        if (wave == (hw >> 1) && hs == (hw & 1)) {
#pragma unroll
            for (int j = 0; j < 8; ++j) {
                float* dg = red + 8 * hl + j;
                dg[0] = (hw > 0 ? dg[0] : 0.f) + dgam[j];
                dg[d] = (hw > 0 ? dg[d] : 0.f) + dbet[j];
            }
        }
        __syncthreads();
    }
    const int n_out = embed_part_elems(d, p.nf);
    float* out = p.part + (int64_t)blockIdx.x * n_out;
    for (int i = threadIdx.x; i < n_out; i += 256) out[i] = i < 2 * d ? red[i] : 0.f;
}

template <typename T> int embed_mix_fwd(const EmbedMix& e, hipStream_t st) {
    if (e.M <= 0) return 0;
    PMGT_CHECK(e.d % 4 == 0 && e.d <= 1024, -2, "embed_mix_fwd: hidden size %d must be a multiple of 4 and <= 1024", e.d);
    if constexpr (sizeof(T) == 2) {
        if (e.phase == 2 && e.d == 256 && e.e_rows != nullptr) {
            PMGT_CHECK(e.S > 0 && e.M % e.S == 0, -2, "embed_mix_fwd: %d tokens are not whole sequences of %d", e.M, e.S);
            const int tasks = tok_tasks(e.M, e.S);
            note_launch(LT_EMBED_TOK8);
            hipLaunchKernelGGL((embed_tok8_fwd_kernel<T>), dim3(cdiv(tasks, 4)), dim3(256), 0, st, e);
            PMGT_LAUNCH_OK();
            return 0;
        }
    }
    PMGT_CHECK(e.phase != 2 || e.pre != nullptr, -2, "embed_mix_fwd: the token phase at hidden size %d stores the pre-LayerNorm sum", e.d);
    PMGT_CHECK(e.nf >= 1 && e.nf <= 4, -2, "embed_mix_fwd: %d modalities (1 .. 4 are built)", e.nf);
    dim3 grid(cdiv(e.M, 4)), block(256);
#define PMGT_EMB_FWD_NF(PH, NF_)                                                                                  \
    do {                                                                                                          \
        if (e.d <= 256) hipLaunchKernelGGL((embed_mix_fwd_kernel<T, 1, PH, NF_>), grid, block, 0, st, e);         \
        else if (e.d <= 512) hipLaunchKernelGGL((embed_mix_fwd_kernel<T, 2, PH, NF_>), grid, block, 0, st, e);    \
        else hipLaunchKernelGGL((embed_mix_fwd_kernel<T, 4, PH, NF_>), grid, block, 0, st, e);                    \
    } while (0)
#define PMGT_EMB_FWD(PH)                                                                                          \
    do {                                                                                                          \
        if (e.nf == 2 || PH == 2) PMGT_EMB_FWD_NF(PH, 2);                                                         \
        else if (e.nf == 1) PMGT_EMB_FWD_NF(PH, 1);                                                               \
        else if (e.nf == 3) PMGT_EMB_FWD_NF(PH, 3);                                                               \
        else PMGT_EMB_FWD_NF(PH, 4);                                                                              \
    } while (0)
    if (e.phase == 1) PMGT_EMB_FWD(1);
    else if (e.phase == 2) PMGT_EMB_FWD(2);
    else PMGT_EMB_FWD(0);
#undef PMGT_EMB_FWD
#undef PMGT_EMB_FWD_NF
    PMGT_LAUNCH_OK();
    return 0;
}
template int embed_mix_fwd<float>(const EmbedMix&, hipStream_t);
template int embed_mix_fwd<bf16>(const EmbedMix&, hipStream_t);

template <typename T, int NCH, int PHASE, int NF>
__global__ __launch_bounds__(256) void embed_mix_bwd_kernel(EmbedMix p) {
    extern __shared__ float red[];
    const int lane = threadIdx.x & 63, wave = threadIdx.x >> 6;
    const int d = p.d, nch = d >> 2;
    const float inv_d = 1.f / (float)d;
    const DropKey ik = make_drop_key(p.drop);
    constexpr int NW = PHASE == 2 ? 1 : NF;
    f32x4 gam[NCH], dgam[NCH], dbet[NCH], dw[NW][NW][NCH], wa[NW][NW][NCH];
    float dba[NW];
#pragma unroll
    for (int k = 0; k < NW; ++k) dba[k] = 0.f;
#pragma unroll
    for (int i = 0; i < NCH; ++i) {
        const int ch = lane + 64 * i;
        const bool ok = ch < nch;
        const f32x4 z = {0.f, 0.f, 0.f, 0.f};
        gam[i] = ok ? *(const f32x4*)(p.gamma + 4 * ch) : z;
        dgam[i] = dbet[i] = z;
#pragma unroll
        for (int k = 0; k < NW; ++k)
#pragma unroll
            for (int f = 0; f < NW; ++f) {
                wa[k][f][i] = (ok && PHASE != 2) ? *(const f32x4*)(p.Wa + ((int64_t)k * NF + f) * d + 4 * ch) : z;
                dw[k][f][i] = z;
            }
    }
    const int rpb = ln_bwd_rows(p.M);
    for (int it = 0; it < rpb / 4; ++it) {
        const int m = blockIdx.x * rpb + it * 4 + wave;
        if (m >= p.M) break;
        f32x4 df[NCH];
        f32x4 ev[NW][NCH];
        if constexpr (PHASE != 2) {
            const T* E = (const T*)p.E + (p.e_rows ? p.e_rows[m] : (int64_t)m) * NF * d;
#pragma unroll
            for (int i = 0; i < NCH; ++i) {
                const int ch = lane + 64 * i;
#pragma unroll
                for (int f = 0; f < NF; ++f) ev[f][i] = ch < nch ? load4<T>(E + f * d + 4 * ch) : (f32x4){0.f, 0.f, 0.f, 0.f};
            }
        }
// ... 185 lines not shown
```

pmgt_amd/csrc/segsum.h:

```cpp
#pragma once
#include "common.h"

namespace pmgt {

int64_t seg_sort_temp_bytes(int M);
int seg_sort(const int64_t* ids, int M, int n_rows, uint32_t* keys, uint32_t* vals, uint32_t* skeys, uint32_t* perm, int* seg_off,
             void* temp, int64_t temp_bytes, hipStream_t st);
int64_t seg_part_elems(int M, int cols);
template <typename T, typename TO>
int seg_sum(const T* src, int64_t ld, const uint32_t* skeys, const uint32_t* perm, const int* seg_off, int M, int n_rows, int cols,
            TO* out, float* part, hipStream_t st);

}
```

pmgt_amd/csrc/segsum.hip:

```cpp
#include <string.h>

#include "segsum.h"

namespace pmgt {

static constexpr int SEG_CH = 64;

static constexpr int RS_ROUNDS = 8, RS_TILE = 256 * RS_ROUNDS, RS_SLOTS = 4 * RS_ROUNDS, RS_MAXBINS = 256;

template <bool FROM_IDS>
__global__ __launch_bounds__(256) void rs_hist_kernel(const int64_t* __restrict__ ids, const uint32_t* __restrict__ kin, int M, int shift, uint32_t mask,
                                                      int ntiles, uint32_t* __restrict__ hist) {
    __shared__ uint32_t h[RS_MAXBINS];
    h[threadIdx.x] = 0;
    __syncthreads();
    const int base = blockIdx.x * RS_TILE;
#pragma unroll 4
    for (int j = 0; j < RS_ROUNDS; ++j) {
        const int idx = base + j * 256 + threadIdx.x;
        if (idx < M) atomicAdd(&h[((FROM_IDS ? (uint32_t)ids[idx] : kin[idx]) >> shift) & mask], 1u);
    }
    __syncthreads();
    if (threadIdx.x <= mask) hist[(int64_t)blockIdx.x * (mask + 1u) + threadIdx.x] = h[threadIdx.x];
}

__global__ __launch_bounds__(256) void rs_colscan_kernel(uint32_t* __restrict__ hist, int ntiles, uint32_t nb, uint32_t* __restrict__ tot) {
    const int lane = threadIdx.x & 63;
    const uint32_t dg = blockIdx.x * 4 + (threadIdx.x >> 6);
    if (dg >= nb) return;
    const int per = (ntiles + 63) / 64, t0 = lane * per, t1 = min(ntiles, t0 + per);
    uint32_t s = 0;
    for (int t = t0; t < t1; ++t) s += hist[(int64_t)t * nb + dg];
    uint32_t inc = s;
#pragma unroll
    for (int o = 1; o < 64; o <<= 1) {
        const uint32_t up = __shfl_up(inc, o, 64);
        if (lane >= o) inc += up;
    }
    uint32_t run = inc - s;
    for (int t = t0; t < t1; ++t) {
        const uint32_t c = hist[(int64_t)t * nb + dg];
        hist[(int64_t)t * nb + dg] = run;
        run += c;
    }
    if (lane == 63) tot[dg] = inc;
}
static constexpr int RS_FOLD_TILES = 256;

template <bool FROM_IDS, bool SCANNED = false>
__global__ __launch_bounds__(256) void rs_scatter_kernel(const int64_t* __restrict__ ids, const uint32_t* __restrict__ kin,
                                                         const uint32_t* __restrict__ vin, int M, int shift, uint32_t mask, int ntiles,
                                                         const uint32_t* __restrict__ base ,
                                                         const uint32_t* __restrict__ coltot ,
                                                         uint32_t* __restrict__ kout, uint32_t* __restrict__ vout) {
    __shared__ uint16_t cnt[RS_MAXBINS][RS_SLOTS + 2];
    __shared__ uint32_t tbase[RS_MAXBINS];
    const int tid = threadIdx.x, lane = tid & 63, wave = tid >> 6, tile = blockIdx.x;
    for (int i = tid; i < RS_MAXBINS * (RS_SLOTS + 2) / 2; i += 256) ((uint32_t*)cnt)[i] = 0u;
    {
        __shared__ uint32_t wtot[4];
        const uint32_t nb = mask + 1u;
        uint32_t tot = 0, pre = 0;
        if (SCANNED) {
            if ((uint32_t)tid < nb) { pre = base[(int64_t)tile * nb + tid]; tot = coltot[tid]; }
        } else if ((uint32_t)tid < nb) {
            uint32_t t0 = 0, t1 = 0, t2 = 0, t3 = 0;
            int t = 0;
            for (; t + 4 <= tile; t += 4) {
                t0 += base[(int64_t)t * nb + tid]; t1 += base[(int64_t)(t + 1) * nb + tid];
                t2 += base[(int64_t)(t + 2) * nb + tid]; t3 += base[(int64_t)(t + 3) * nb + tid];
            }
            for (; t < tile; ++t) t0 += base[(int64_t)t * nb + tid];
            pre = t0 + t1 + t2 + t3;
            t0 = t1 = t2 = t3 = 0;
            for (; t + 4 <= ntiles; t += 4) {
                t0 += base[(int64_t)t * nb + tid]; t1 += base[(int64_t)(t + 1) * nb + tid];
                t2 += base[(int64_t)(t + 2) * nb + tid]; t3 += base[(int64_t)(t + 3) * nb + tid];
            }
            for (; t < ntiles; ++t) t0 += base[(int64_t)t * nb + tid];
            tot = pre + t0 + t1 + t2 + t3;
        }
        uint32_t inc = tot;
#pragma unroll
        for (int o = 1; o < 64; o <<= 1) {
            const uint32_t up = __shfl_up(inc, o, 64);
            if (lane >= o) inc += up;
        }
        if (lane == 63) wtot[wave] = inc;
        __syncthreads();
// ... 136 lines not shown
#pragma unroll
            for (int g = 0; g < CG; ++g) {
                const int col = 2 * (tid + 256 * g);
                if (col < cols) { acc[g][0] += pr[col]; acc[g][1] += pr[col + 1]; }
            }
        }
    }
#pragma unroll
    for (int g = 0; g < CG; ++g) {
        const int col = 2 * (tid + 256 * g);
        if (col < cols) {
            out[(int64_t)k * cols + col] = (T)acc[g][0];
            out[(int64_t)k * cols + col + 1] = (T)acc[g][1];
        }
    }
}

static inline int rs_tiles(int M) { return cdiv(M, RS_TILE); }

int64_t seg_sort_temp_bytes(int M) {
    return (int64_t)RS_MAXBINS * rs_tiles(M) * 4 + 256 + RS_MAXBINS * 4;
}

int seg_sort(const int64_t* ids, int M, int n_rows, uint32_t* keys, uint32_t* vals, uint32_t* skeys, uint32_t* perm, int* seg_off,
             void* temp, int64_t temp_bytes, hipStream_t st) {
    PMGT_CHECK(M > 0 && n_rows > 0, -2, "seg_sort: empty input");
    PMGT_CHECK(temp_bytes >= seg_sort_temp_bytes(M), -4, "seg_sort: temporary storage too small (%lld > %lld)", (long long)seg_sort_temp_bytes(M),
               (long long)temp_bytes);
    int bits = 1;
    while ((1ll << bits) < (int64_t)n_rows) ++bits;
    const int passes = cdiv(bits, 8), w = cdiv(bits, passes);
    const int ntiles = rs_tiles(M);
    uint32_t* hist[1] = {(uint32_t*)temp};
    uint32_t* coltot = (uint32_t*)((char*)temp + (int64_t)RS_MAXBINS * ntiles * 4 + 256);
    const uint32_t mask = (1u << w) - 1u;
    const uint32_t *kin = nullptr, *vin = nullptr;
    for (int p = 0; p < passes; ++p) {
        uint32_t* kout = ((passes - 1 - p) & 1) ? keys : skeys;
        uint32_t* vout = ((passes - 1 - p) & 1) ? vals : perm;
        const int shift = p * w;
        if (p == 0) hipLaunchKernelGGL(rs_hist_kernel<true>, dim3(ntiles), dim3(256), 0, st, ids, kin, M, shift, mask, ntiles, hist[0]);
        else hipLaunchKernelGGL(rs_hist_kernel<false>, dim3(ntiles), dim3(256), 0, st, ids, kin, M, shift, mask, ntiles, hist[0]);
        if (ntiles > RS_FOLD_TILES) {
            hipLaunchKernelGGL(rs_colscan_kernel, dim3(cdiv((int)mask + 1, 4)), dim3(256), 0, st, hist[0], ntiles, mask + 1u, coltot);
            if (p == 0) hipLaunchKernelGGL((rs_scatter_kernel<true, true>), dim3(ntiles), dim3(256), 0, st, ids, kin, vin, M, shift, mask, ntiles, hist[0], coltot, kout, vout);
            else hipLaunchKernelGGL((rs_scatter_kernel<false, true>), dim3(ntiles), dim3(256), 0, st, ids, kin, vin, M, shift, mask, ntiles, hist[0], coltot, kout, vout);
        } else {
            if (p == 0) hipLaunchKernelGGL((rs_scatter_kernel<true, false>), dim3(ntiles), dim3(256), 0, st, ids, kin, vin, M, shift, mask, ntiles, hist[0], coltot, kout, vout);
            else hipLaunchKernelGGL((rs_scatter_kernel<false, false>), dim3(ntiles), dim3(256), 0, st, ids, kin, vin, M, shift, mask, ntiles, hist[0], coltot, kout, vout);
        }
        kin = kout; vin = vout;
    }
    PMGT_LAUNCH_OK();
    hipLaunchKernelGGL(seg_bounds_kernel, dim3(cdiv(M, 256)), dim3(256), 0, st, skeys, M, n_rows, seg_off);
    PMGT_LAUNCH_OK();
    return 0;
}

int64_t seg_part_elems(int M, int cols) { return (int64_t)cdiv(M, SEG_CH) * 2 * cols; }

template <typename T, typename TO>
int seg_sum(const T* src, int64_t ld, const uint32_t* skeys, const uint32_t* perm, const int* seg_off, int M, int n_rows, int cols,
            TO* out, float* part, hipStream_t st) {
    PMGT_CHECK(cols % 4 == 0 && cols <= 1024 && ld % 4 == 0, -2, "seg_sum: cols=%d must be a multiple of 4 and <= 1024", cols);
    const int chunks = cdiv(cdiv(M, SEG_CH), 4);
    const int cg = cdiv(cols, 256);
    switch (cg) {
        case 1:
            hipLaunchKernelGGL((seg_sum_kernel<T, TO, 1>), dim3(chunks), dim3(256), 0, st, src, ld, skeys, perm, seg_off, M, cols, out, part);
            hipLaunchKernelGGL((seg_fix_kernel<TO, 1>), dim3(n_rows), dim3(256), 0, st, seg_off, n_rows, cols, part, out);
            break;
        case 2:
            hipLaunchKernelGGL((seg_sum_kernel<T, TO, 2>), dim3(chunks), dim3(256), 0, st, src, ld, skeys, perm, seg_off, M, cols, out, part);
            hipLaunchKernelGGL((seg_fix_kernel<TO, 2>), dim3(n_rows), dim3(256), 0, st, seg_off, n_rows, cols, part, out);
            break;
        default:
            hipLaunchKernelGGL((seg_sum_kernel<T, TO, 4>), dim3(chunks), dim3(256), 0, st, src, ld, skeys, perm, seg_off, M, cols, out, part);
            hipLaunchKernelGGL((seg_fix_kernel<TO, 4>), dim3(n_rows), dim3(256), 0, st, seg_off, n_rows, cols, part, out);
            break;
    }
    PMGT_LAUNCH_OK();
    return 0;
}
template int seg_sum<float, float>(const float*, int64_t, const uint32_t*, const uint32_t*, const int*, int, int, int, float*, float*, hipStream_t);
template int seg_sum<bf16, bf16>(const bf16*, int64_t, const uint32_t*, const uint32_t*, const int*, int, int, int, bf16*, float*, hipStream_t);
template int seg_sum<bf16, float>(const bf16*, int64_t, const uint32_t*, const uint32_t*, const int*, int, int, int, float*, float*, hipStream_t);

}
```

pmgt_amd/ops/row_ops.hip:

```cpp
#include <vector>

#include "../../include/pmgt_ops.h"
#include "../csrc/loss.h"
#include "../csrc/optim.h"
#include "../csrc/rowops.h"
#include "../csrc/segsum.h"

using namespace pmgt;

extern "C" {

static EmbedMix mk_embed(const pmgt_embed_args* a) {
    EmbedMix m;
    m.M = a->M; m.S = a->S; m.d = a->d; m.nf = a->nf; m.E = a->E; m.e_rows = a->e_rows; m.phase = a->phase; m.dF_f32 = a->dF_f32 != 0;
    m.Wa = a->Wa; m.ba = a->ba; m.pos = a->pos; m.role = a->role; m.gamma = a->gamma; m.beta = a->beta; m.eps = a->eps;
    m.a = a->a; m.pre = a->pre; m.stats = a->stats; m.h0 = a->h0;
    m.drop = DropCfg{a->rng, a->rng ? a->drop_p : 0.f, a->drop_site};
    m.dh0 = a->dh0; m.dE = a->dE; m.dF = a->dF; m.part = a->part;
    return m;
}
int pmgt_op_embed_mix_fwd(const pmgt_embed_args* a, void* stream) {
    PMGT_CHECK(a && a->phase >= 0 && a->phase <= 2, -2, "pmgt_op_embed_mix_fwd: phase must be 0, 1 or 2");
    const EmbedMix m = mk_embed(a);
    if (a->dtype == PMGT_DTYPE_BF16) return embed_mix_fwd<bf16>(m, (hipStream_t)stream);
    return embed_mix_fwd<float>(m, (hipStream_t)stream);
}
int pmgt_op_embed_mix_bwd(const pmgt_embed_args* a, void* stream) {
    PMGT_CHECK(a && a->phase >= 0 && a->phase <= 2, -2, "pmgt_op_embed_mix_bwd: phase must be 0, 1 or 2");
    const EmbedMix m = mk_embed(a);
    if (a->dtype == PMGT_DTYPE_BF16) return embed_mix_bwd<bf16>(m, (hipStream_t)stream);
    return embed_mix_bwd<float>(m, (hipStream_t)stream);
}
int pmgt_op_embed_part_elems(int d, int nf) { return embed_part_elems(d, nf); }
int pmgt_op_embed_bwd_parts(int M) { return embed_bwd_parts(M); }
int pmgt_op_pos_role_finish(const float* possum, int S, int d, int max_pos, float* dpos, float* drole, int accumulate, void* stream) {
    return pos_role_finish(possum, S, d, max_pos, dpos, drole, accumulate != 0, (hipStream_t)stream);
}

int64_t pmgt_op_seg_part_elems(int M, int cols) { return seg_part_elems(M, cols); }
int pmgt_op_seg_sum(int in_dtype, int out_dtype, const void* src, int64_t ld, const uint32_t* skeys, const uint32_t* perm, const int* seg_off,
                    int M, int n_rows, int cols, void* out, float* part, void* stream) {
    const hipStream_t st = (hipStream_t)stream;
    if (in_dtype == PMGT_DTYPE_F32 && out_dtype == PMGT_DTYPE_F32)
        return seg_sum<float, float>((const float*)src, ld, skeys, perm, seg_off, M, n_rows, cols, (float*)out, part, st);
    if (in_dtype == PMGT_DTYPE_BF16 && out_dtype == PMGT_DTYPE_BF16)
        return seg_sum<bf16, bf16>((const bf16*)src, ld, skeys, perm, seg_off, M, n_rows, cols, (bf16*)out, part, st);
    PMGT_CHECK(in_dtype == PMGT_DTYPE_BF16 && out_dtype == PMGT_DTYPE_F32, -2, "pmgt_op_seg_sum: dtype pair (%d, %d) is not built", in_dtype,
               out_dtype);
    return seg_sum<bf16, float>((const bf16*)src, ld, skeys, perm, seg_off, M, n_rows, cols, (float*)out, part, st);
}

int pmgt_op_pair_offsets(const int64_t* num_pairs, int B, int* off, void* stream) {
    return pair_offsets(num_pairs, B, off, (hipStream_t)stream);
}
int pmgt_op_nfr_compact(const int64_t* tgt_full, int B, int S, int seq_off, int64_t* rows, int64_t* tids, int* count, void* stream) {
    return nfr_compact(tgt_full, B, S, seq_off, rows, tids, count, (hipStream_t)stream);
}
int pmgt_op_nfr_generate(const int64_t* ids, int B, int S, int n_nodes, float random_ratio, float mask_ratio, const uint64_t* rng,
                         int64_t* masked_ids, int64_t* tgt_full, void* stream) {
    PMGT_CHECK(ids && rng && masked_ids && tgt_full && B > 0 && S > 0 && n_nodes > 0, -2, "pmgt_op_nfr_generate: NULL or empty argument");
    return nfr_generate(ids, B, S, n_nodes, random_ratio, mask_ratio, rng, masked_ids, tgt_full, (hipStream_t)stream);
}
int pmgt_op_build_need_rows(int B, int P, int S, const int64_t* nfr_rows, const int* nfr_count, int64_t* rows, int* count, int* inv,
                            int64_t n_tokens, void* stream) {
    PMGT_CHECK(nfr_rows && nfr_count && rows && count && B > 0 && P >= 0 && S > 0, -2, "pmgt_op_build_need_rows: NULL or empty argument");
    return build_need_rows(B, P, S, nfr_rows, nfr_count, rows, count, (hipStream_t)stream, inv, n_tokens);
}
int pmgt_op_gsr(int dtype, const void* h, void* dh, int B, int S, int d, int64_t cls_stride, const int* off, const float* labels,
                float* logits, float* loss_part, void* stream) {
    GsrArgs g;
    g.h = h; g.dh = dh; g.B = B; g.S = S; g.d = d; g.cls_stride = cls_stride; g.off = off; g.labels = labels; g.logits = logits;
    g.loss_part = loss_part;
    if (dtype == PMGT_DTYPE_BF16) return gsr_fwd_bwd<bf16>(g, (hipStream_t)stream);
    return gsr_fwd_bwd<float>(g, (hipStream_t)stream);
}
int pmgt_op_nfr_diff_parts(int cap) { return nfr_diff_parts(cap); }
int pmgt_op_nfr_diff(int dtype, void* pred, const int64_t* tids, const int* count, int cap, int nf, const int* F, const void* const* tables,
                     int tables_f8, const float* scales, float* sse_part, void* stream) {
    PMGT_CHECK(nf >= 1 && nf <= MAX_FEATS && F && tables, -2, "pmgt_op_nfr_diff: %d modalities (1 .. %d)", nf, MAX_FEATS);
    NfrDiffArgs a;
    a.pred = pred; a.tids = tids; a.count = count; a.cap = cap; a.nf = nf; a.tables_f8 = tables_f8 != 0; a.sse_part = sse_part;
    for (int m = 0; m < nf; ++m) { a.F[m] = F[m]; a.table[m] = tables[m]; a.scale[m] = scales ? scales[m] : 1.f; }
    if (dtype == PMGT_DTYPE_BF16) return nfr_diff<bf16>(a, (hipStream_t)stream);
    return nfr_diff<float>(a, (hipStream_t)stream);
}
int pmgt_op_loss_finish(const float* gsr_part, int B, const float* sse_part, int nparts, const int* count, int nf, const int* F, int with_nfr,
                        float* out, int* count_out, void* stream) {
    PMGT_CHECK(nf >= 1 && nf <= MAX_FEATS && F, -2, "pmgt_op_loss_finish: %d modalities (1 .. %d)", nf, MAX_FEATS);
    FeatSizes fs;
    fs.nf = nf;
    for (int m = 0; m < MAX_FEATS; ++m) fs.F[m] = m < nf ? F[m] : 0;
    return loss_finish(gsr_part, B, sse_part, nparts, count, fs, with_nfr != 0, out, (hipStream_t)stream, count_out);
}
int pmgt_op_scatter_rows(int dtype, const void* src, const int64_t* rows, const int* count, int cap, int d, void* dst, int add, void* stream) {
    if (dtype == PMGT_DTYPE_BF16) return scatter_rows<bf16>((const bf16*)src, rows, count, cap, d, (bf16*)dst, (hipStream_t)stream, add != 0);
    return scatter_rows<float>((const float*)src, rows, count, cap, d, (float*)dst, (hipStream_t)stream, add != 0);
}

static int mirror_from_host(int dtype, const float* params, void* mirror, const MirrorDesc* h, MirrorDesc* dev, int ndesc, int total_tiles,
                            hipStream_t st) {
    PMGT_HIP(hipMemcpyAsync(dev, h, sizeof(MirrorDesc) * (size_t)ndesc, hipMemcpyHostToDevice, st));
    const int rc = dtype == PMGT_DTYPE_BF16 ? build_mirror<bf16>(params, (bf16*)mirror, dev, ndesc, total_tiles, st)
                                            : build_mirror<float>(params, (float*)mirror, dev, ndesc, total_tiles, st);
    if (rc) return rc;
    PMGT_HIP(hipStreamSynchronize(st));
    return 0;
}
int pmgt_op_mirror(int dtype, const float* params, void* mirror, const pmgt_mirror_desc* desc, int ndesc, int total_tiles, void* stream) {
    PMGT_CHECK(desc && ndesc > 0, -2, "pmgt_op_mirror: no descriptors");
    std::vector<MirrorDesc> h((size_t)ndesc);
    for (int k = 0; k < ndesc; ++k) {
        const pmgt_mirror_desc& s = desc[k];
        h[k] = MirrorDesc{s.src, s.rows, s.cols, s.dst, s.dst_t, s.dst_t_hm, s.hm_d, s.hm_dh, s.tile_start};
    }
// ... 11 lines not shown
```

Measured before the change: 108,800 target nodes/s.

## Fuse embedding LayerNorm backward with sorted segment sum and position colsum

Adds a sorted-order embedding backward kernel that walks tokens in node-sorted order. In one pass it computes the LayerNorm backward, accumulates per-node segment sums, and accumulates position gradients in LDS. This replaces the separate embed_mix_bwd, colsum and seg_sum launches, along with the extra write and reread of the token gradient buffer. In exchange it adds a larger LDS footprint, a seg_fix pass for segments that cross block boundaries, and gathered (permuted) reads of the token inputs.

```diff
diff --git a/include/pmgt_ops.h b/include/pmgt_ops.h
--- a/include/pmgt_ops.h
+++ b/include/pmgt_ops.h
@@ -30,6 +30,7 @@
 #define PMGT_OPT_NO_CLS_ONLY_ATTENTION_BWD (1u << 21)
 #define PMGT_OPT_NO_BETA_SKIP (1u << 22)
 #define PMGT_OPT_NO_VC2_ATTENTION_BWD (1u << 23)
+#define PMGT_OPT_NO_SORTED_EMBED_BWD (1u << 24)
 #define PMGT_OPT_NO_TILE_ATTENTION (1u << 17)
 
 void pmgt_launch_trace_reset(void);
@@ -122,6 +123,9 @@
 } pmgt_embed_args;
 int pmgt_op_embed_mix_fwd(const pmgt_embed_args* args, void* stream);
 int pmgt_op_embed_mix_bwd(const pmgt_embed_args* args, void* stream);
+int pmgt_op_embed_sorted_parts(int M);
+int pmgt_op_embed_tok8_bwd_sorted(const pmgt_embed_args* args, const uint32_t* skeys, const uint32_t* perm, const int* seg_off, int n_rows,
+                                  float* node_sums, float* seg_part, float* pos_part, void* stream);
 int pmgt_op_embed_part_elems(int d, int nf);
 int pmgt_op_embed_bwd_parts(int M);
 int pmgt_op_pos_role_finish(const float* possum, int S, int d, int max_pos, float* dpos, float* drole, int accumulate, void* stream);
diff --git a/pmgt_amd/_lib.py b/pmgt_amd/_lib.py
--- a/pmgt_amd/_lib.py
+++ b/pmgt_amd/_lib.py
@@ -175,12 +175,13 @@
     "pmgt_op_adamw_scheduled", "pmgt_op_lr_schedule", "pmgt_op_nfr_generate", "pmgt_op_build_need_rows", "pmgt_op_dropout_keep",
     "pmgt_op_adamw_guarded", "pmgt_op_eval_append_scores", "pmgt_op_eval_small_max",
     "pmgt_op_linear_rows", "pmgt_op_layernorm_bwd_rows", "pmgt_op_gemm_tn_bias_rows",
+    "pmgt_op_embed_tok8_bwd_sorted", "pmgt_op_embed_sorted_parts",
     "pmgt_op_adamw_segments", "pmgt_op_cls_gather", "pmgt_op_cls_scatter", "pmgt_op_sgd", "pmgt_op_step_segments",
 ]
 OPT = {k: 1 << i for i, k in enumerate((
     "tile_gemm", "valu_attention", "wave_attention_bwd", "no_shortcut", "no_fused_qkvc_attention", "no_head_major",
     "no_table_projection", "no_segment_sum", "consumer_quant", "no_fused_attention_bwd", "store_ln_input", "eager_reduce",
-    "side_stream_reduce", "unfused_ln", "one_bucket", "small_arena", "no_role_split_ln", "no_tile_attention", "unfused_ln_bwd", "lockstep_attention_bwd", "side_stream_wgrad", "no_cls_only_attention_bwd", "no_beta_skip", "no_vc2_attention_bwd"))}
+    "side_stream_reduce", "unfused_ln", "one_bucket", "small_arena", "no_role_split_ln", "no_tile_attention", "unfused_ln_bwd", "lockstep_attention_bwd", "side_stream_wgrad", "no_cls_only_attention_bwd", "no_beta_skip", "no_vc2_attention_bwd", "no_sorted_embed_bwd"))}
 SAMPLER_SYMBOLS = [
     "pmgt_sampler_create", "pmgt_sampler_destroy", "pmgt_sampler_last_error", "pmgt_sampler_seed",
     "pmgt_sampler_context", "pmgt_sampler_batch", "pmgt_sampler_batch_mt", "pmgt_sampler_max_pairs",
@@ -274,6 +275,8 @@
     L.pmgt_op_qkvc_attention_fwd_f8.argtypes = [vp, vp, vp, vp, vp, vp, vp, vp, vp, i, i, i, i, f, f, u32, u32, vp, vp]
     L.pmgt_op_embed_mix_fwd.argtypes = [C.POINTER(EmbedArgsC), vp]
     L.pmgt_op_embed_mix_bwd.argtypes = [C.POINTER(EmbedArgsC), vp]
+    L.pmgt_op_embed_tok8_bwd_sorted.argtypes = [C.POINTER(EmbedArgsC), vp, vp, vp, i, vp, vp, vp, vp]
+    L.pmgt_op_embed_sorted_parts.argtypes = [i]
     L.pmgt_op_embed_part_elems.argtypes = [i, i]
     L.pmgt_op_embed_bwd_parts.argtypes = [i]
     L.pmgt_op_pos_role_finish.argtypes = [vp, i, i, i, vp, vp, i, vp]
diff --git a/pmgt_amd/csrc/common.h b/pmgt_amd/csrc/common.h
--- a/pmgt_amd/csrc/common.h
+++ b/pmgt_amd/csrc/common.h
@@ -56,7 +56,7 @@
 enum LaunchTag {
     LT_GEMM_WSR = 0, LT_GEMM_WSR_LNB, LT_GEMM_WSR512, LT_GEMM_WS, LT_NT_BIG, LT_NT_BIG_GATHER, LT_NT_BIG_128, LT_NT_LNB, LT_NT_TILE,
     LT_TN_BIG, LT_TN_BIG_GATHER, LT_TN_DMA, LT_TN_DMA_GATHER, LT_TN_TILE, LT_ATTN_TILES_FWD, LT_ATTN_TILES_BWD, LT_QKVC_ATTN_FWD,
-    LT_ATTN_BWD_WGRAD, LT_F8_BIG, LT_F8_TILE, LT_F8_WSR512, LT_GEMM_ROWLN, LT_NT_LNF, LT_EMBED_TOK8, LT_QKVC_ATTN_FWD_VC, LT_ATTN_BWD_WGRAD_VC, LT_NT_VC, LT_ATTN_BWD_WGRAD_VC2, LT_COUNT
+    LT_ATTN_BWD_WGRAD, LT_F8_BIG, LT_F8_TILE, LT_F8_WSR512, LT_GEMM_ROWLN, LT_NT_LNF, LT_EMBED_TOK8, LT_QKVC_ATTN_FWD_VC, LT_ATTN_BWD_WGRAD_VC, LT_NT_VC, LT_ATTN_BWD_WGRAD_VC2, LT_EMBED_TOK8_SORTED, LT_COUNT
 };
 void note_launch(int tag);
 
@@ -274,6 +274,7 @@
     OPT_NO_CLS_ONLY_ATTENTION_BWD = 1u << 21,
     OPT_NO_BETA_SKIP = 1u << 22,
     OPT_NO_VC2_ATTENTION_BWD = 1u << 23,
+    OPT_NO_SORTED_EMBED_BWD = 1u << 24,
     OPT_SIDE_STREAM_WGRAD = 1u << 20,
 };
 
diff --git a/pmgt_amd/csrc/engine.hip b/pmgt_amd/csrc/engine.hip
--- a/pmgt_amd/csrc/engine.hip
+++ b/pmgt_amd/csrc/engine.hip
@@ -30,7 +30,7 @@
 static const char* const g_launch_names[LT_COUNT] = {
     "gemm_wsr", "gemm_wsr_lnb", "gemm_wsr512", "gemm_ws", "nt_big", "nt_big_gather", "nt_big_128", "nt_lnb", "nt_tile",
     "tn_big", "tn_big_gather", "tn_dma", "tn_dma_gather", "tn_tile", "attn_tiles_fwd", "attn_tiles_bwd", "qkvc_attn_fwd",
-    "attn_bwd_wgrad", "f8_big", "f8_tile", "f8_wsr512", "gemm_rowln", "nt_lnf", "embed_tok8", "qkvc_attn_fwd_vc", "attn_bwd_wgrad_vc", "nt_vc", "attn_bwd_wgrad_vc2"};
+    "attn_bwd_wgrad", "f8_big", "f8_tile", "f8_wsr512", "gemm_rowln", "nt_lnf", "embed_tok8", "qkvc_attn_fwd_vc", "attn_bwd_wgrad_vc", "nt_vc", "attn_bwd_wgrad_vc2", "embed_tok8_sorted"};
 
 static inline int64_t align_up(int64_t x, int64_t a) { return (x + a - 1) / a * a; }
 
@@ -362,6 +362,7 @@
     part = std::max(part, colsum_slab_elems((int)M, std::max(I, 4 * d)));
     part = std::max(part, colsum_slab_elems(Tseq, S * d));
     part = std::max(part, colsum_slab_elems(cap, F));
+    part = std::max(part, align_up((int64_t)embed_sorted_parts((int)M) * embed_part_elems(d, NF), 64) + (int64_t)embed_sorted_parts((int)M) * S * d);
     part = std::max(part, (int64_t)512 * std::max(std::max(I, 4 * d), F));
     b.part = c.get<float>(part);
     b.part_side_elems = (int64_t)512 * std::max(std::max(I, 4 * d), F);
@@ -488,6 +489,11 @@
 template <typename T>
 static inline bool embed_recomputes(const pmgt_engine* e, bool table_mode) {
     return table_mode && !(e->opts & OPT_NO_SEGMENT_SUM) && e->d == 256 && sizeof(T) == 2;
+}
+
+template <typename T>
+static inline bool embed_sorted_applies(const pmgt_engine* e, int S) {
+    return embed_recomputes<T>(e, true) && !e->fp8 && !(e->opts & OPT_NO_SORTED_EMBED_BWD) && embed_sorted_fits(S);
 }
 
 template <typename T>
@@ -1028,15 +1034,36 @@
             if (embed_recomputes<T>(e, true)) {
                 m.pre = nullptr; m.E = b.E + (int64_t)n_rows * NF * d; m.e_rows = b.ids; m.pos = P + e->pos; m.role = P + e->role;
             }
-            if (b.defer) RUN(take_partials<T>(e, b, (int64_t)embed_bwd_parts(M) * pe, &m.part, st));
-            RUNP("bwd.embed_mix", embed_mix_bwd<T>(m, st));
-            if (b.defer) RUN(queue_reduce<T>(e, b, m.part, embed_bwd_parts(M), pe, G + e->ln_g, acc, st));
-            else RUNP("bwd.slab_reduce", slab_reduce(b.part, embed_bwd_parts(M), pe, G + e->ln_g, acc, st));
-            RUNP("bwd.colsum", colsum<T>(b.bB, (int64_t)S * d, Tseq, S * d, b.part, b.possum, false, nullptr, st));
-            RUN(pos_role_finish(b.possum, S, d, e->cfg.max_position_embeddings, G + e->pos, G + e->role, acc, st));
-            if (b.sort_done) PMGT_HIP(hipStreamWaitEvent(st, b.sort_done, 0));
-            else RUNP("bwd.segsum_featproj", seg_sort(b.ids, M, n_rows, b.sg_keys, b.sg_vals, b.sg_skeys, b.sg_perm, b.sg_off, b.sg_tmp, b.sg_tmp_bytes, st));
-            RUNP("bwd.segsum_featproj", (seg_sum<T, float>(b.bB, d, b.sg_skeys, b.sg_perm, b.sg_off, M, n_rows, d, (float*)b.bC, b.sg_part, st)));
+            if (embed_sorted_applies<T>(e, S)) {
+                if (b.sort_done) PMGT_HIP(hipStreamWaitEvent(st, b.sort_done, 0));
+                else RUNP("bwd.segsum_featproj", seg_sort(b.ids, M, n_rows, b.sg_keys, b.sg_vals, b.sg_skeys, b.sg_perm, b.sg_off, b.sg_tmp, b.sg_tmp_bytes, st));
+                const int parts = embed_sorted_parts(M);
+                EmbedSorted q;
+                q.skeys = b.sg_skeys; q.perm = b.sg_perm; q.seg_off = b.sg_off; q.out = (float*)b.bC; q.part = b.sg_part;
+                if (b.defer) RUN(take_partials2<T>(e, b, (int64_t)parts * pe, &m.part, (int64_t)parts * S * d, &q.pos_part, st));
+                else q.pos_part = b.part + align_up((int64_t)parts * pe, 64);
+                RUNP("bwd.embed_mix", embed_tok8_bwd_sorted<T>(m, q, st));
+                if (b.defer) {
+                    RUN(queue_reduce<T>(e, b, m.part, parts, pe, G + e->ln_g, acc, st));
+                    RUN(queue_reduce<T>(e, b, q.pos_part, parts, (int64_t)S * d, b.possum, false, st));
+                    RUN(flush_reduces<T>(e, b, st));
+                } else {
+                    RUNP("bwd.slab_reduce", slab_reduce(b.part, parts, pe, G + e->ln_g, acc, st));
+                    RUNP("bwd.slab_reduce", slab_reduce(q.pos_part, parts, (int64_t)S * d, b.possum, false, st));
+                }
+                RUN(pos_role_finish(b.possum, S, d, e->cfg.max_position_embeddings, G + e->pos, G + e->role, acc, st));
+                RUNP("bwd.segsum_featproj", seg_fix<float>(b.sg_off, n_rows, d, b.sg_part, (float*)b.bC, st));
+            } else {
+                if (b.defer) RUN(take_partials<T>(e, b, (int64_t)embed_bwd_parts(M) * pe, &m.part, st));
+                RUNP("bwd.embed_mix", embed_mix_bwd<T>(m, st));
+                if (b.defer) RUN(queue_reduce<T>(e, b, m.part, embed_bwd_parts(M), pe, G + e->ln_g, acc, st));
+                else RUNP("bwd.slab_reduce", slab_reduce(b.part, embed_bwd_parts(M), pe, G + e->ln_g, acc, st));
+                RUNP("bwd.colsum", colsum<T>(b.bB, (int64_t)S * d, Tseq, S * d, b.part, b.possum, false, nullptr, st));
+                RUN(pos_role_finish(b.possum, S, d, e->cfg.max_position_embeddings, G + e->pos, G + e->role, acc, st));
+                if (b.sort_done) PMGT_HIP(hipStreamWaitEvent(st, b.sort_done, 0));
+                else RUNP("bwd.segsum_featproj", seg_sort(b.ids, M, n_rows, b.sg_keys, b.sg_vals, b.sg_skeys, b.sg_perm, b.sg_off, b.sg_tmp, b.sg_tmp_bytes, st));
+                RUNP("bwd.segsum_featproj", (seg_sum<T, float>(b.bB, d, b.sg_skeys, b.sg_perm, b.sg_off, M, n_rows, d, (float*)b.bC, b.sg_part, st)));
+            }
             m.phase = 1; m.M = n_rows; m.E = b.E; m.e_rows = nullptr; m.dF = b.bC; m.dF_f32 = true; m.dE = b.bD;
             m.part = b.part;
             if (b.defer) RUN(take_partials<T>(e, b, (int64_t)embed_bwd_parts(n_rows) * pe, &m.part, st));
@@ -1547,7 +1574,7 @@
               PMGT_OPT_NO_SHORTCUT == OPT_NO_SHORTCUT && PMGT_OPT_NO_FUSED_QKVC_ATTENTION == OPT_NO_FUSED_QKVC_ATTENTION && PMGT_OPT_NO_HEAD_MAJOR == OPT_NO_HEAD_MAJOR &&
               PMGT_OPT_NO_TABLE_PROJECTION == OPT_NO_TABLE_PROJECTION && PMGT_OPT_NO_SEGMENT_SUM == OPT_NO_SEGMENT_SUM && PMGT_OPT_CONSUMER_QUANT == OPT_CONSUMER_QUANT &&
               PMGT_OPT_NO_FUSED_ATTENTION_BWD == OPT_NO_FUSED_ATTENTION_BWD && PMGT_OPT_STORE_LN_INPUT == OPT_STORE_LN_INPUT && PMGT_OPT_EAGER_REDUCE == OPT_EAGER_REDUCE &&
-              PMGT_OPT_SIDE_STREAM_REDUCE == OPT_SIDE_STREAM_REDUCE && PMGT_OPT_UNFUSED_LN == OPT_UNFUSED_LN && PMGT_OPT_ONE_BUCKET == OPT_ONE_BUCKET && PMGT_OPT_SMALL_ARENA == OPT_SMALL_ARENA && PMGT_OPT_NO_ROLE_SPLIT_LN == OPT_NO_ROLE_SPLIT_LN && PMGT_OPT_NO_TILE_ATTENTION == OPT_NO_TILE_ATTENTION,
+              PMGT_OPT_SIDE_STREAM_REDUCE == OPT_SIDE_STREAM_REDUCE && PMGT_OPT_UNFUSED_LN == OPT_UNFUSED_LN && PMGT_OPT_ONE_BUCKET == OPT_ONE_BUCKET && PMGT_OPT_SMALL_ARENA == OPT_SMALL_ARENA && PMGT_OPT_NO_ROLE_SPLIT_LN == OPT_NO_ROLE_SPLIT_LN && PMGT_OPT_NO_TILE_ATTENTION == OPT_NO_TILE_ATTENTION && PMGT_OPT_NO_SORTED_EMBED_BWD == OPT_NO_SORTED_EMBED_BWD,
               "include/pmgt_ops.h and csrc/common.h disagree on the option bits");
 static uint32_t option_bit(const char* key) {
     static const struct { const char* name; uint32_t bit; } tab[] = {
@@ -1555,7 +1582,7 @@
         {"no_shortcut", OPT_NO_SHORTCUT}, {"no_fused_qkvc_attention", OPT_NO_FUSED_QKVC_ATTENTION}, {"no_head_major", OPT_NO_HEAD_MAJOR},
         {"no_table_projection", OPT_NO_TABLE_PROJECTION}, {"no_segment_sum", OPT_NO_SEGMENT_SUM}, {"consumer_quant", OPT_CONSUMER_QUANT},
         {"no_fused_attention_bwd", OPT_NO_FUSED_ATTENTION_BWD}, {"store_ln_input", OPT_STORE_LN_INPUT}, {"eager_reduce", OPT_EAGER_REDUCE},
-        {"side_stream_reduce", OPT_SIDE_STREAM_REDUCE}, {"unfused_ln", OPT_UNFUSED_LN}, {"one_bucket", OPT_ONE_BUCKET}, {"small_arena", OPT_SMALL_ARENA}, {"no_role_split_ln", OPT_NO_ROLE_SPLIT_LN}, {"no_tile_attention", OPT_NO_TILE_ATTENTION}, {"unfused_ln_bwd", OPT_UNFUSED_LN_BWD}, {"lockstep_attention_bwd", OPT_LOCKSTEP_ATTENTION_BWD}, {"side_stream_wgrad", OPT_SIDE_STREAM_WGRAD}, {"no_cls_only_attention_bwd", OPT_NO_CLS_ONLY_ATTENTION_BWD}, {"no_beta_skip", OPT_NO_BETA_SKIP}, {"no_vc2_attention_bwd", OPT_NO_VC2_ATTENTION_BWD}};
+        {"side_stream_reduce", OPT_SIDE_STREAM_REDUCE}, {"unfused_ln", OPT_UNFUSED_LN}, {"one_bucket", OPT_ONE_BUCKET}, {"small_arena", OPT_SMALL_ARENA}, {"no_role_split_ln", OPT_NO_ROLE_SPLIT_LN}, {"no_tile_attention", OPT_NO_TILE_ATTENTION}, {"unfused_ln_bwd", OPT_UNFUSED_LN_BWD}, {"lockstep_attention_bwd", OPT_LOCKSTEP_ATTENTION_BWD}, {"side_stream_wgrad", OPT_SIDE_STREAM_WGRAD}, {"no_cls_only_attention_bwd", OPT_NO_CLS_ONLY_ATTENTION_BWD}, {"no_beta_skip", OPT_NO_BETA_SKIP}, {"no_vc2_attention_bwd", OPT_NO_VC2_ATTENTION_BWD}, {"no_sorted_embed_bwd", OPT_NO_SORTED_EMBED_BWD}};
     for (const auto& t : tab)
         if (key && strcmp(key, t.name) == 0) return t.bit;
     return 0;
diff --git a/pmgt_amd/csrc/rowops.h b/pmgt_amd/csrc/rowops.h
--- a/pmgt_amd/csrc/rowops.h
+++ b/pmgt_amd/csrc/rowops.h
@@ -42,6 +42,19 @@
 template <typename T> int embed_mix_fwd(const EmbedMix& e, hipStream_t st);
 template <typename T> int embed_mix_bwd(const EmbedMix& e, hipStream_t st);
 inline int embed_bwd_parts(int M) { return cdiv(M, ln_bwd_rows(M)); }
+struct EmbedSorted {
+    const uint32_t* skeys = nullptr;
+    const uint32_t* perm = nullptr;
+    const int* seg_off = nullptr;
+    float* out = nullptr;
+    float* part = nullptr;
+    float* pos_part = nullptr;
+};
+constexpr int EMBED_SORTED_MAX_S = 38;
+inline int64_t embed_sorted_lds_bytes(int S) { return ((int64_t)1024 * S + 1536) * 4; }
+inline bool embed_sorted_fits(int S) { return S >= 1 && S <= EMBED_SORTED_MAX_S; }
+inline int embed_sorted_parts(int M) { const int g = cdiv(cdiv(M, 64), 8); return g < 256 ? g : 256; }
+template <typename T> int embed_tok8_bwd_sorted(const EmbedMix& e, const EmbedSorted& q, hipStream_t st);
 int pos_role_finish(const float* possum, int S, int d, int max_pos, float* dpos, float* drole, bool accumulate,
                     hipStream_t st);
 
diff --git a/pmgt_amd/csrc/rowops.hip b/pmgt_amd/csrc/rowops.hip
--- a/pmgt_amd/csrc/rowops.hip
+++ b/pmgt_amd/csrc/rowops.hip
@@ -1,5 +1,6 @@
 #include "fp8.h"
 #include "rowops.h"
+#include "segsum.h"
 
 namespace pmgt {
 
@@ -483,6 +484,44 @@
     }
 }
 
+__device__ __forceinline__ bf16x8 tok_ln_bwd_row(const bf16x8& x, const f32x4 (&ps)[2], const f32x4 (&rl)[2], const bf16x8& dy, bool ok, float mean,
+                                                 float rstd, uint32_t m, int hl, const DropKey& ik, const f32x4 (&gam)[2], float (&dgam)[8],
+                                                 float (&dbet)[8]) {
+    constexpr int d = 256;
+    float v[8], g[8], dyv[8];
+    tok_sum(x, ps, rl, v);
+#pragma unroll
+    for (int j = 0; j < 8; ++j) dyv[j] = ok ? (float)dy[j] : 0.f;
+    if (ik.on) {
+#pragma unroll
+        for (int c = 0; c < 2; ++c) {
+            float dm[4];
+            drop_mul4(ik, m, (uint32_t)(2 * hl + c), dm);
+#pragma unroll
+            for (int e = 0; e < 4; ++e) dyv[4 * c + e] *= dm[e];
+        }
+    }
+    bf16x8 o;
+    {
+#pragma clang fp contract(off)
+        float sg = 0.f, sgx = 0.f;
+#pragma unroll
+        for (int j = 0; j < 8; ++j) {
+            v[j] = ((float)(bf16)v[j] - mean) * rstd;
+            g[j] = dyv[j] * gam[j >> 2][j & 3];
+            dgam[j] = __builtin_fmaf(dyv[j], v[j], dgam[j]);
+            dbet[j] += dyv[j];
+            sg = __builtin_fmaf(dyv[j], gam[j >> 2][j & 3], sg);
+            sgx = __builtin_fmaf(v[j], g[j], sgx);
+        }
+        sg = half_sum(sg);
+        sgx = half_sum(sgx) * (1.f / (float)d);
+#pragma unroll
+        for (int j = 0; j < 8; ++j) o[j] = (bf16)(__builtin_fmaf(-v[j], sgx, __builtin_fmaf(sg, -1.f / (float)d, g[j])) * rstd);
+    }
+    return o;
+}
+
 template <typename T>
 __global__ __launch_bounds__(256) void embed_tok8_bwd_kernel(EmbedMix p) {
     static_assert(sizeof(T) == 2, "bf16 only");
@@ -523,34 +562,7 @@
         for (int k = 0; k < R; ++k) {
             const bool ok = tk.sv && tk.q0 + k < Tq;
             const int64_t m = (int64_t)min(tk.q0 + k, Tq - 1) * S + tk.s;
-            float v[8], g[8], dyv[8];
-            tok_sum(x[k], ps, rl, v);
-#pragma unroll
-            for (int j = 0; j < 8; ++j) dyv[j] = ok ? (float)dy[k][j] : 0.f;
-            if (ik.on) {
-#pragma unroll
-                for (int c = 0; c < 2; ++c) {
-                    float dm[4];
-                    drop_mul4(ik, (uint32_t)m, (uint32_t)(2 * hl + c), dm);
-#pragma unroll
-                    for (int e = 0; e < 4; ++e) dyv[4 * c + e] *= dm[e];
-                }
-            }
-            float sg = 0.f, sgx = 0.f;
-#pragma unroll
-            for (int j = 0; j < 8; ++j) {
-                v[j] = ((float)(bf16)v[j] - mean[k]) * rstd[k];
-                g[j] = dyv[j] * gam[j >> 2][j & 3];
-                dgam[j] += dyv[j] * v[j];
-                dbet[j] += dyv[j];
-                sg += g[j];
-                sgx += g[j] * v[j];
-            }
-            sg = half_sum(sg) * (1.f / (float)d);
-            sgx = half_sum(sgx) * (1.f / (float)d);
-            bf16x8 o;
-#pragma unroll
-            for (int j = 0; j < 8; ++j) o[j] = (bf16)((g[j] - sg - v[j] * sgx) * rstd[k]);
+            const bf16x8 o = tok_ln_bwd_row(x[k], ps, rl, dy[k], ok, mean[k], rstd[k], (uint32_t)m, hl, ik, gam, dgam, dbet);
             if (ok) *(bf16x8*)((bf16*)p.dF + m * d + 8 * hl) = o;
         }
     }
@@ -569,6 +581,187 @@
     float* out = p.part + (int64_t)blockIdx.x * n_out;
     for (int i = threadIdx.x; i < n_out; i += 256) out[i] = i < 2 * d ? red[i] : 0.f;
 }
+
+constexpr int SRT_U = 4;
+struct SrtBatch {
+    bf16x8 dy[SRT_U], x[SRT_U];
+    f32x4 ps[SRT_U][2];
+    float mean[SRT_U], rstd[SRT_U];
+    uint32_t m[SRT_U], key[SRT_U];
+    int s[SRT_U];
+};
+template <typename T>
+__global__ __launch_bounds__(256) void embed_tok8_bwd_sorted_kernel(EmbedMix p, EmbedSorted q) {
+    static_assert(sizeof(T) == 2, "bf16 only");
+    extern __shared__ float smem[];
+    constexpr int d = 256;
+    const int lane = threadIdx.x & 63, hl = lane & 31, hs = lane >> 5, wave = threadIdx.x >> 6;
+    const int S = p.S, M = p.M;
+    const bool s_pow2 = (S & (S - 1)) == 0;
+    float* const slab = smem + (int64_t)wave * S * d;
+    uint32_t* const sk = (uint32_t*)(smem + 4 * S * d) + (wave * 2 + hs) * 2 * SEG_CH;
+    uint32_t* const sp = sk + SEG_CH;
+    float* const red = smem + 4 * S * d + 16 * SEG_CH;
+    for (int i = threadIdx.x * 4; i < 4 * S * d; i += 1024) *(f32x4*)(smem + i) = (f32x4){0.f, 0.f, 0.f, 0.f};
+    __syncthreads();
+    const DropKey ik = make_drop_key(p.drop);
+    f32x4 gam[2], rl0[2], rl1[2];
+#pragma unroll
+    for (int c = 0; c < 2; ++c) {
+        gam[c] = *(const f32x4*)(p.gamma + 8 * hl + 4 * c);
+        rl0[c] = *(const f32x4*)(p.role + 8 * hl + 4 * c);
+        rl1[c] = *(const f32x4*)(p.role + d + 8 * hl + 4 * c);
+    }
+    float dgam[8], dbet[8], acc[8];
+#pragma unroll
+    for (int j = 0; j < 8; ++j) dgam[j] = dbet[j] = acc[j] = 0.f;
+    const int nchunks = (M + SEG_CH - 1) / SEG_CH, npairs = (nchunks + 1) >> 1;
+    const int wstep = gridDim.x * 4;
+    uint32_t nk[2], np[2], nk_before = 0xffffffffu, nk_behind = 0xffffffffu;
+    auto fetch_keys = [&](int w) {
+        const int c0 = (2 * w + hs) * SEG_CH;
+#pragma unroll
+        for (int r = 0; r < 2; ++r) {
+            const int pp = min(c0 + hl + 32 * r, M - 1);
+            nk[r] = q.skeys[pp];
+            np[r] = q.perm[pp];
+        }
+        nk_before = c0 > 0 && c0 <= M ? q.skeys[c0 - 1] : 0xffffffffu;
+        nk_behind = c0 + SEG_CH < M ? q.skeys[c0 + SEG_CH] : 0xffffffffu;
+    };
+    auto load_batch = [&](SrtBatch& B, int i0) {
+#pragma unroll
+        for (int u = 0; u < SRT_U; ++u) {
+            B.m[u] = sp[i0 + u];
+            B.key[u] = sk[i0 + u];
+            B.s[u] = s_pow2 ? (int)(B.m[u] & (uint32_t)(S - 1)) : (int)(B.m[u] % (uint32_t)S);
+        }
+#pragma unroll
+        for (int u = 0; u < SRT_U; ++u) {
+            const int64_t m = B.m[u];
+            B.dy[u] = *(const bf16x8*)((const bf16*)p.dh0 + m * d + 8 * hl);
+            const float2 st = *(const float2*)(p.stats + 2 * m);
+            B.mean[u] = st.x;
+            B.rstd[u] = st.y;
+#pragma unroll
+            for (int c = 0; c < 2; ++c) B.ps[u][c] = *(const f32x4*)(p.pos + (int64_t)B.s[u] * d + 8 * hl + 4 * c);
+            B.x[u] = *(const bf16x8*)((const bf16*)p.E + (int64_t)B.key[u] * d + 8 * hl);
+        }
+    };
+    int w = blockIdx.x * 4 + wave;
+    if (w < npairs) fetch_keys(w);
+    for (; w < npairs; w += wstep) {
+        const int chunk = 2 * w + hs, p0 = chunk * SEG_CH;
+        const int n = max(0, min(SEG_CH, M - p0));
+        const int n_wave = min(SEG_CH, M - 2 * w * SEG_CH);
+#pragma unroll
+        for (int r = 0; r < 2; ++r) { sk[hl + 32 * r] = nk[r]; sp[hl + 32 * r] = np[r]; }
+        __builtin_amdgcn_wave_barrier();
+        const uint32_t k_before = nk_before, k_behind = nk_behind;
+        if (w + wstep < npairs) fetch_keys(w + wstep);
+        int a = p0;
+        uint32_t cur = sk[0];
+        auto flush = [&](int b) {
+            const bool complete = (a > p0 || k_before != cur) && (b < p0 + n || k_behind != cur);
+            float* dst = complete ? q.out + (int64_t)cur * d : q.part + ((int64_t)chunk * 2 + (a == p0 ? 0 : 1)) * d;
+            *(f32x4*)(dst + 8 * hl) = (f32x4){acc[0], acc[1], acc[2], acc[3]};
+            *(f32x4*)(dst + 8 * hl + 4) = (f32x4){acc[4], acc[5], acc[6], acc[7]};
+#pragma unroll
+            for (int j = 0; j < 8; ++j) acc[j] = 0.f;
+        };
+        auto work = [&](const SrtBatch& B, int i0) {
+#pragma unroll
+            for (int u = 0; u < SRT_U; ++u) {
+                const int i = i0 + u;
+                const bool ok = i < n;
+                const int s = B.s[u];
+                const f32x4 rl[2] = {s > 0 ? rl1[0] : rl0[0], s > 0 ? rl1[1] : rl0[1]};
+                const bf16x8 o = tok_ln_bwd_row(B.x[u], B.ps[u], rl, B.dy[u], ok, B.mean[u], B.rstd[u], B.m[u], hl, ik, gam, dgam, dbet);
+                float of[8];
+#pragma unroll
+                for (int j = 0; j < 8; ++j) of[j] = (float)o[j];
+                if (ok) {
+                    if (B.key[u] != cur) {
+                        flush(p0 + i);
+                        a = p0 + i;
+                        cur = B.key[u];
+                    }
+#pragma unroll
+                    for (int j = 0; j < 8; ++j) acc[j] += of[j];
+                }
+                float* sl = slab + s * d + 4 * hl;
+                auto add_pos = [&]() {
+                    f32x4 t0 = *(f32x4*)sl, t1 = *(f32x4*)(sl + 128);
+                    t0 += (f32x4){of[0], of[1], of[2], of[3]};
+                    t1 += (f32x4){of[4], of[5], of[6], of[7]};
+                    *(f32x4*)sl = t0;
+                    *(f32x4*)(sl + 128) = t1;
+                };
+                const int s_lo = __builtin_amdgcn_readlane(s, 0), s_hi = __builtin_amdgcn_readlane(s, 32);
+                if (s_lo != s_hi) {
+                    if (ok) add_pos();
+                } else {
+                    if (hs == 0 && ok) add_pos();
+                    if (hs == 1 && ok) add_pos();
+                }
+            }
+        };
+        SrtBatch B0, B1;
+        load_batch(B0, 0);
+#pragma unroll 1
+        for (int i0 = 0; i0 < n_wave; i0 += 2 * SRT_U) {
+            load_batch(B1, i0 + SRT_U);
+            work(B0, i0);
+            if (i0 + 2 * SRT_U < SEG_CH) load_batch(B0, i0 + 2 * SRT_U);
+            work(B1, i0 + SRT_U);
+        }
+        if (n > 0) flush(p0 + n);
+        __builtin_amdgcn_wave_barrier();
+    }
+    for (int hw = 0; hw < 8; ++hw) {
+        if (wave == (hw >> 1) && hs == (hw & 1)) {
+#pragma unroll
+            for (int j = 0; j < 8; ++j) {
+                float* dg = red + 8 * hl + j;
+                dg[0] = (hw > 0 ? dg[0] : 0.f) + dgam[j];
+                dg[d] = (hw > 0 ? dg[d] : 0.f) + dbet[j];
+            }
+        }
+        __syncthreads();
+    }
+    const int n_out = embed_part_elems(d, p.nf);
+    float* out = p.part + (int64_t)blockIdx.x * n_out;
+    for (int i = threadIdx.x; i < n_out; i += 256) out[i] = i < 2 * d ? red[i] : 0.f;
+    float* pp = q.pos_part + (int64_t)blockIdx.x * S * d;
+    for (int i = threadIdx.x * 4; i < S * d; i += 1024) {
+        f32x4 v = *(const f32x4*)(smem + i);
+#pragma unroll
+        for (int k = 1; k < 4; ++k) v += *(const f32x4*)(smem + (int64_t)k * S * d + i);
+        const int s = i >> 8, c = (i >> 7) & 1, l = (i >> 2) & 31;
+        *(f32x4*)(pp + s * d + 8 * l + 4 * c) = v;
+    }
+}
+
+template <typename T> int embed_tok8_bwd_sorted(const EmbedMix& e, const EmbedSorted& q, hipStream_t st) {
+    if constexpr (sizeof(T) == 2) {
+        PMGT_CHECK(e.M > 0 && e.d == 256 && e.S > 0 && e.M % e.S == 0 && embed_sorted_fits(e.S), -2,
+                   "embed_tok8_bwd_sorted: needs hidden size 256 and whole sequences of at most %d positions (d=%d, S=%d, M=%d)", EMBED_SORTED_MAX_S, e.d,
+                   e.S, e.M);
+        PMGT_CHECK(e.nf >= 1 && e.nf <= 4, -2, "embed_tok8_bwd_sorted: %d modalities (1 .. 4 are built)", e.nf);
+        PMGT_CHECK(e.E && e.pos && e.role && e.gamma && e.stats && e.dh0 && e.part && q.skeys && q.perm && q.seg_off && q.out && q.part && q.pos_part, -2,
+                   "embed_tok8_bwd_sorted: NULL operand");
+        const int lds = (int)embed_sorted_lds_bytes(e.S);
+        PMGT_SMEM_ATTR((const void*)embed_tok8_bwd_sorted_kernel<T>, (int)embed_sorted_lds_bytes(EMBED_SORTED_MAX_S));
+        note_launch(LT_EMBED_TOK8);
+        note_launch(LT_EMBED_TOK8_SORTED);
+        hipLaunchKernelGGL((embed_tok8_bwd_sorted_kernel<T>), dim3(embed_sorted_parts(e.M)), dim3(256), lds, st, e, q);
+        PMGT_LAUNCH_OK();
+        return 0;
+    }
+    PMGT_CHECK(false, -2, "embed_tok8_bwd_sorted: bf16 only");
+}
+template int embed_tok8_bwd_sorted<float>(const EmbedMix&, const EmbedSorted&, hipStream_t);
+template int embed_tok8_bwd_sorted<bf16>(const EmbedMix&, const EmbedSorted&, hipStream_t);
 
 template <typename T> int embed_mix_fwd(const EmbedMix& e, hipStream_t st) {
     if (e.M <= 0) return 0;
diff --git a/pmgt_amd/csrc/segsum.h b/pmgt_amd/csrc/segsum.h
--- a/pmgt_amd/csrc/segsum.h
+++ b/pmgt_amd/csrc/segsum.h
@@ -6,7 +6,10 @@
 int64_t seg_sort_temp_bytes(int M);
 int seg_sort(const int64_t* ids, int M, int n_rows, uint32_t* keys, uint32_t* vals, uint32_t* skeys, uint32_t* perm, int* seg_off,
              void* temp, int64_t temp_bytes, hipStream_t st);
+constexpr int SEG_CH = 64;
 int64_t seg_part_elems(int M, int cols);
+template <typename TO>
+int seg_fix(const int* seg_off, int n_rows, int cols, const float* part, TO* out, hipStream_t st);
 template <typename T, typename TO>
 int seg_sum(const T* src, int64_t ld, const uint32_t* skeys, const uint32_t* perm, const int* seg_off, int M, int n_rows, int cols,
             TO* out, float* part, hipStream_t st);
diff --git a/pmgt_amd/csrc/segsum.hip b/pmgt_amd/csrc/segsum.hip
--- a/pmgt_amd/csrc/segsum.hip
+++ b/pmgt_amd/csrc/segsum.hip
@@ -3,8 +3,6 @@
 #include "segsum.h"
 
 namespace pmgt {
-
-static constexpr int SEG_CH = 64;
 
 static constexpr int RS_ROUNDS = 8, RS_TILE = 256 * RS_ROUNDS, RS_SLOTS = 4 * RS_ROUNDS, RS_MAXBINS = 256;
 
@@ -307,6 +305,18 @@
     PMGT_LAUNCH_OK();
     return 0;
 }
+template <typename TO>
+int seg_fix(const int* seg_off, int n_rows, int cols, const float* part, TO* out, hipStream_t st) {
+    PMGT_CHECK(cols % 4 == 0 && cols <= 1024 && n_rows > 0, -2, "seg_fix: cols=%d must be a multiple of 4 and <= 1024", cols);
+    const int cg = cdiv(cols, 256);
+    if (cg == 1) hipLaunchKernelGGL((seg_fix_kernel<TO, 1>), dim3(n_rows), dim3(256), 0, st, seg_off, n_rows, cols, part, out);
+    else if (cg == 2) hipLaunchKernelGGL((seg_fix_kernel<TO, 2>), dim3(n_rows), dim3(256), 0, st, seg_off, n_rows, cols, part, out);
+    else hipLaunchKernelGGL((seg_fix_kernel<TO, 4>), dim3(n_rows), dim3(256), 0, st, seg_off, n_rows, cols, part, out);
+    PMGT_LAUNCH_OK();
+    return 0;
+}
+template int seg_fix<float>(const int*, int, int, const float*, float*, hipStream_t);
+
 template int seg_sum<float, float>(const float*, int64_t, const uint32_t*, const uint32_t*, const int*, int, int, int, float*, float*, hipStream_t);
 template int seg_sum<bf16, bf16>(const bf16*, int64_t, const uint32_t*, const uint32_t*, const int*, int, int, int, bf16*, float*, hipStream_t);
 template int seg_sum<bf16, float>(const bf16*, int64_t, const uint32_t*, const uint32_t*, const int*, int, int, int, float*, float*, hipStream_t);
diff --git a/pmgt_amd/ops/row_ops.hip b/pmgt_amd/ops/row_ops.hip
--- a/pmgt_amd/ops/row_ops.hip
+++ b/pmgt_amd/ops/row_ops.hip
@@ -30,6 +30,19 @@
     const EmbedMix m = mk_embed(a);
     if (a->dtype == PMGT_DTYPE_BF16) return embed_mix_bwd<bf16>(m, (hipStream_t)stream);
     return embed_mix_bwd<float>(m, (hipStream_t)stream);
+}
+int pmgt_op_embed_sorted_parts(int M) { return embed_sorted_parts(M); }
+int pmgt_op_embed_tok8_bwd_sorted(const pmgt_embed_args* a, const uint32_t* skeys, const uint32_t* perm, const int* seg_off, int n_rows,
+                                  float* node_sums, float* seg_part, float* pos_part, void* stream) {
+    PMGT_CHECK(a && skeys && perm && seg_off && node_sums && seg_part && pos_part && n_rows > 0, -2, "pmgt_op_embed_tok8_bwd_sorted: NULL or empty argument");
+    PMGT_CHECK(a->dtype == PMGT_DTYPE_BF16 && a->phase == 2 && a->pre == nullptr, -2,
+               "pmgt_op_embed_tok8_bwd_sorted: the bf16 token phase with the recomputed pre-LayerNorm sum only");
+    EmbedMix m = mk_embed(a);
+    EmbedSorted q;
+    q.skeys = skeys; q.perm = perm; q.seg_off = seg_off; q.out = node_sums; q.part = seg_part; q.pos_part = pos_part;
+    const int rc = embed_tok8_bwd_sorted<bf16>(m, q, (hipStream_t)stream);
+    if (rc) return rc;
+    return seg_fix<float>(seg_off, n_rows, a->d, seg_part, node_sums, (hipStream_t)stream);
 }
 int pmgt_op_embed_part_elems(int d, int nf) { return embed_part_elems(d, nf); }
 int pmgt_op_embed_bwd_parts(int M) { return embed_bwd_parts(M); }
```

New measurement: 107,600 target nodes/s. -1.1%, worse.
